# gooofy/zerovox

Hardware: AMD Instinct MI355X
Metric: audio samples/sec + RTF, 128-phoneme zero-shot synth @22.05kHz, 1/2/4/8 GPU (higher is better)
Workload: dtype f16+bf16

## Files before the change

### zerovox_amd/csrc/gemm.hip

```cpp
#include "mfma_util.h"
#include "zvx_kernels.h"

#include <cstring>
#include <type_traits>

#ifndef ZVX_GEMM_PART
#define ZVX_GEMM_PART 0
#endif
#define ZVX_PART_MAIN (ZVX_GEMM_PART != 2)
#define ZVX_PART_RESFUSE (ZVX_GEMM_PART != 1)
#if ZVX_GEMM_PART == 2
extern thread_local bool zvx_gemm_dry_run;
#else
thread_local hipEvent_t zvx_gemm_ev_start = nullptr, zvx_gemm_ev_stop = nullptr;
thread_local bool zvx_gemm_dry_run = false;
#endif
#define g_dry_run zvx_gemm_dry_run

#define ZVX_LAUNCH(...) do { if (!g_dry_run) ZVX_DISPATCH(__VA_ARGS__); } while (0)

namespace zvx {


#define PITCH 80
// ... 102 lines not shown
                }
            }
        }
    }
}

template <int DT, int BM, int BN, int WM, int WN>
__global__ __launch_bounds__(256) void gemm_kernel(const GemmArgs a) {
    constexpr int ES = (DT == DT_F32) ? 4 : 2;
    constexpr int EPC = 16 / ES;
    constexpr int BKE = KBYTES / ES;
    constexpr int TM = BM / WM / 32, TN = BN / WN / 32;
    constexpr int XCH = BM * 4 / 256;
    constexpr int WCH = (BN * 4 + 255) / 256;
    static_assert(WM * WN == 4, "4 waves");

    __shared__ __attribute__((aligned(16))) unsigned char lds[2][(BM + BN) * PITCH];

    const int tid = threadIdx.x, lane = tid & 63, wave = tid >> 6;
    const int wr = wave % WM, wc = wave / WM;

    const int ntn = (a.N + BN - 1) / BN;
    const int nwg = gridDim.x;
    int wg;
    {
        const int id = blockIdx.x, q = nwg >> 3, r = nwg & 7, xcd = id & 7;
        wg = (xcd < r ? xcd * (q + 1) : r * (q + 1) + (xcd - r) * q) + (id >> 3);
    }
    const int nt = wg % ntn, mt = wg / ntn;
    const int m0 = mt * BM, n0 = nt * BN;
    const int z = blockIdx.y, b = z / a.nheads, h = z - b * a.nheads;

    const int out_len = a.out_len ? a.out_len[b] : a.M;
    const int in_len = a.in_len ? a.in_len[b] : a.in_len_static;
    const bool two_d = a.wout > 0;
    if (!two_d && m0 >= out_len) return;
    if (m0 >= a.M) return;
    int Kb = a.K;
    if (a.k_len) { Kb = (a.k_len[b] + 7) & ~7; if (Kb > a.K) Kb = a.K; }

    const unsigned char* Xp = (const unsigned char*)a.X + ((long)b * a.x_bs + (long)h * a.x_hs) * ES;
    const unsigned char* Wp = (const unsigned char*)a.W + ((long)b * a.w_bs + (long)h * a.w_hs) * ES;

    int xu[XCH], xv[XCH];
    const int kc = tid & 3;
#pragma unroll
    for (int i = 0; i < XCH; i++) {
        const int r = m0 + (tid >> 2) + i * 64;
        if (two_d) { xu[i] = (r / a.wout) * a.stride; xv[i] = (r % a.wout) * a.stride; }
        else { xu[i] = 0; xv[i] = r; }
    }

    const int kchunks = (Kb + BKE - 1) / BKE;
    const int S = a.ntaps * kchunks;

    uint4 xreg[XCH], wreg[WCH];

    auto load_regs = [&](int s) {
        const int tap = s / kchunks;
        const int k = (s - tap * kchunks) * BKE + kc * EPC;
        const bool kok = k < Kb;
        const int du = a.du[tap], dv = a.dv[tap];
#pragma unroll
        for (int i = 0; i < XCH; i++) {
            const int iu = xu[i] + du, iv = xv[i] + dv;
            const bool ok = kok && iu >= 0 && iu < a.hin && iv >= 0 && iv < in_len;
            uint4 v = make_uint4(0, 0, 0, 0);
            if (ok) v = *(const uint4*)(Xp + ((long)(iu * a.win + iv) * a.ldx + k) * ES);
            xreg[i] = v;
        }
#pragma unroll
        for (int i = 0; i < WCH; i++) {
            const int c = tid + i * 256;
            const int n = n0 + (c >> 2);
            uint4 v = make_uint4(0, 0, 0, 0);
            if ((BN * 4 >= 256 * (i + 1) || c < BN * 4) && kok && n < a.N)
                v = *(const uint4*)(Wp + ((long)tap * a.w_ts + (long)n * a.ldw + k) * ES);
            wreg[i] = v;
        }
    };
    auto store_lds = [&](int buf) {
        unsigned char* base = lds[buf];
#pragma unroll
        for (int i = 0; i < XCH; i++)
            *(uint4*)(base + ((tid >> 2) + i * 64) * PITCH + kc * 16) = xreg[i];
#pragma unroll
        for (int i = 0; i < WCH; i++) {
            const int c = tid + i * 256;
            if (BN * 4 >= 256 * (i + 1) || c < BN * 4)
                *(uint4*)(base + (BM + (c >> 2)) * PITCH + kc * 16) = wreg[i];
        }
    };

    f32x16 acc[TN][TM];
#pragma unroll
    for (int i = 0; i < TN; i++)
#pragma unroll
        for (int j = 0; j < TM; j++)
#pragma unroll
            for (int e = 0; e < 16; e++) acc[i][j][e] = 0.f;

    const int xrow = wr * (BM / WM) + (lane & 31);
    const int wrow = BM + wc * (BN / WN) + (lane & 31);
    const int koff = (lane >> 5) * 16;

    if (S > 0) {
        load_regs(0);
        store_lds(0);
    }
    __syncthreads();
    for (int s = 0; s < S; s++) {
        if (s + 1 < S) load_regs(s + 1);
        const unsigned char* base = lds[s & 1];
#pragma unroll
        for (int sub = 0; sub < 2; sub++) {
            uint4 xf[TM], wf[TN];
#pragma unroll
            for (int j = 0; j < TM; j++) xf[j] = *(const uint4*)(base + (xrow + j * 32) * PITCH + sub * 32 + koff);
#pragma unroll
            for (int i = 0; i < TN; i++) wf[i] = *(const uint4*)(base + (wrow + i * 32) * PITCH + sub * 32 + koff);
#pragma unroll
            for (int i = 0; i < TN; i++)
#pragma unroll
                for (int j = 0; j < TM; j++) {
                    if (DT == DT_BF16) {
                        acc[i][j] = __builtin_amdgcn_mfma_f32_32x32x16_bf16(
                            __builtin_bit_cast(bf16x8, wf[i]), __builtin_bit_cast(bf16x8, xf[j]), acc[i][j], 0, 0, 0);
                    } else if (DT == DT_F16) {
                        acc[i][j] = __builtin_amdgcn_mfma_f32_32x32x16_f16(
                            __builtin_bit_cast(f16x8, wf[i]), __builtin_bit_cast(f16x8, xf[j]), acc[i][j], 0, 0, 0);
                    } else {
                        acc[i][j] = __builtin_amdgcn_mfma_f32_32x32x2f32(__uint_as_float(wf[i].x), __uint_as_float(xf[j].x), acc[i][j], 0, 0, 0);
                        acc[i][j] = __builtin_amdgcn_mfma_f32_32x32x2f32(__uint_as_float(wf[i].y), __uint_as_float(xf[j].y), acc[i][j], 0, 0, 0);
                        acc[i][j] = __builtin_amdgcn_mfma_f32_32x32x2f32(__uint_as_float(wf[i].z), __uint_as_float(xf[j].z), acc[i][j], 0, 0, 0);
                        acc[i][j] = __builtin_amdgcn_mfma_f32_32x32x2f32(__uint_as_float(wf[i].w), __uint_as_float(xf[j].w), acc[i][j], 0, 0, 0);
                    }
                }
        }
        if (s + 1 < S) store_lds((s + 1) & 1);
        __syncthreads();
    }

    epilogue<TM, TN>(a, acc, b, h, m0 + wr * (BM / WM), n0 + wc * (BN / WN), out_len, two_d, lane);
}

__device__ __forceinline__ unsigned pack_f16x2(float lo, float hi) { return pack_f16x2_sat(lo, hi); }
__device__ __forceinline__ unsigned pack16x2(float lo, float hi, bool f16) { return f16 ? pack_f16x2_sat(lo, hi) : pack_bf16x2(lo, hi); }
__device__ __forceinline__ f32x2 unpack16x2(unsigned u, bool f16) { return f16 ? unpack_f16x2(u) : unpack_bf16x2(u); }

#define ZVX_EPI(res, am, out) ((res) | ((am) << 1) | ((out) << 3))
#define ZVX_EPI_DEC(res) (16 | 8 | (res))
#define ZVX_EPI_FLIP (ZVX_EPI(0, 0, 1) | 32)

template <int TM, int TN, int RES_LDS = 0, int EPI = -1, bool H16 = false>
__device__ __forceinline__ void epilogue_rows(const GemmArgs& a, f32x16 (&acc)[TN][TM], int b, int row_base, int col_base,
                                              int out_len, int lane, unsigned char* stage ,
                                              const unsigned char* res_lds = nullptr ,
                                              int res_pitch = 0) {
    constexpr int NW = TN * 32;
    constexpr int EP = NW * 4 + 16;
    constexpr int LPR = NW / 8;
    constexpr int RPP = 64 / LPR;
    constexpr int NP = 32 / RPP;
    constexpr bool CT = EPI >= 0;
    constexpr bool DEC = CT && (EPI & 16) != 0;
    constexpr bool BURST = !(CT && !DEC && ((EPI >> 1) & 1));
    const long ooff = (long)b * a.o_bs, roff = (long)b * a.r_bs, aoff = (long)b * a.a_bs;
    const int c8 = lane % LPR;
    const int n = col_base + c8 * 8;
    const bool nok = n < a.N;
    const float alpha = CT ? 1.f : a.alpha, oscale = a.out_scale, rinv = a.res_inv_slope;
    const int act = DEC ? ACT_NONE : (CT ? ACT_LRELU : a.act);
    const float slope = CT ? (a.act == ACT_LRELU ? a.slope : 1.f) : a.slope;
    const int res_mode = RES_LDS ? 2 : (DEC ? (EPI & 1) : (CT ? ((EPI & 1) ? 2 : 0) : a.res_mode));
    const int accum_mode = DEC ? 0 : (CT ? (EPI >> 1) & 3 : a.accum_mode), bias_mode = (CT && !DEC) ? 1 : a.bias_mode;
    const bool has_out = CT ? (EPI >> 3) & 1 : a.out != nullptr, out_bf16 = CT || a.out_dtype != DT_F32, has_post = !CT && a.post_scale != nullptr;
    const bool out_f16 = CT ? H16 : a.out_dtype == DT_F16, res_f16 = (CT || RES_LDS) ? H16 : a.res_dtype == DT_F16, acc_f16 = CT ? H16 : ((TN == 1 || TM <= 2) && a.accum_dtype == DT_F16);
    const bool acc_bf16 = CT || a.accum_dtype == DT_BF16 || acc_f16, res_bf16 = CT || RES_LDS || a.res_dtype != DT_F32;
#define pk2(lo, hi, f16) ((CT && H16) ? pack_f16x2_raw(lo, hi) : pack16x2(lo, hi, f16))
    f32x2 bcol[4];
#pragma unroll
    for (int e = 0; e < 4; e++) bcol[e] = (f32x2){0.f, 0.f};
    if (bias_mode == 1 && nok) {
        const float4 b0 = *(const float4*)(a.bias + n), b1 = *(const float4*)(a.bias + n + 4);
        bcol[0] = (f32x2){b0.x, b0.y}; bcol[1] = (f32x2){b0.z, b0.w}; bcol[2] = (f32x2){b1.x, b1.y}; bcol[3] = (f32x2){b1.z, b1.w};
    }
    u32x4 pk[TM][NP];
    const bool res_glb = !RES_LDS && res_mode && res_bf16;
    uint4 rnext[NP];
    auto res_prefetch = [&](int j) {
#pragma unroll
        for (int p = 0; p < NP; p++) {
            const int r = row_base + j * 32 + p * RPP + lane / LPR;
            const bool okp = r < a.M && r < out_len && nok;
            rnext[p] = *(const uint4*)((const unsigned short*)a.res + (okp ? roff + (long)r * a.ldr + n : 0));
        }
    };
    if (res_glb) res_prefetch(0);
#pragma unroll
    for (int j = 0; j < TM; j++) {
#pragma unroll
        for (int i = 0; i < TN; i++)
#pragma unroll
            for (int g = 0; g < 4; g++)
                *(float4*)(stage + (lane & 31) * EP + (i * 32 + 8 * g + 4 * (lane >> 5)) * 4) =
                    make_float4(acc[i][j][4 * g], acc[i][j][4 * g + 1], acc[i][j][4 * g + 2], acc[i][j][4 * g + 3]);
        f32x2 v[NP][4];
        uint4 rraw[NP];
        float4 aa0[NP], aa1[NP];
        uint4 aab[NP];
        bool ok[NP];
        if (res_glb) {
#pragma unroll
            for (int p = 0; p < NP; p++) rraw[p] = rnext[p];
            if (j + 1 < TM) res_prefetch(j + 1);
        }
#pragma unroll
        for (int p = 0; p < NP; p++) {
            const int rl = p * RPP + lane / LPR;
            const int r = row_base + j * 32 + rl;
            ok[p] = r < a.M && r < out_len && nok;
            const float4 v0 = *(const float4*)(stage + rl * EP + c8 * 32), v1 = *(const float4*)(stage + rl * EP + c8 * 32 + 16);
            v[p][0] = (f32x2){v0.x, v0.y}; v[p][1] = (f32x2){v0.z, v0.w}; v[p][2] = (f32x2){v1.x, v1.y}; v[p][3] = (f32x2){v1.z, v1.w};
            if (RES_LDS == 1) rraw[p] = *(const uint4*)(res_lds + (j * 32 + rl) * res_pitch + (col_base + c8 * 8) * 2);
            if (accum_mode & 1) {
                const long ai = ok[p] ? aoff + (long)r * a.lda + n : 0;
                if (acc_bf16) aab[p] = *(const uint4*)((const unsigned short*)a.accum + ai);
                else { const float* ap = (const float*)a.accum + ai; aa0[p] = *(const float4*)ap; aa1[p] = *(const float4*)(ap + 4); }
            }
        }
#pragma unroll
        for (int p = 0; p < NP; p++) {
            const int r = row_base + j * 32 + p * RPP + lane / LPR;
            f32x2* t = v[p];
            if (alpha != 1.f) {
#pragma unroll
                for (int e = 0; e < 4; e++) t[e] *= alpha;
            }
            if (bias_mode == 1) {
#pragma unroll
                for (int e = 0; e < 4; e++) t[e] += bcol[e];
            } else if (bias_mode == 2) {
                const float brow = ok[p] ? a.bias[r] : 0.f;
#pragma unroll
                for (int e = 0; e < 4; e++) t[e] += brow;
            }
            if (res_mode) {
                f32x2 q[4];
                if (res_bf16) {
                    q[0] = unpack16x2(rraw[p].x, res_f16); q[1] = unpack16x2(rraw[p].y, res_f16); q[2] = unpack16x2(rraw[p].z, res_f16); q[3] = unpack16x2(rraw[p].w, res_f16);
                } else {
                    const float* rp = (const float*)a.res + (ok[p] ? roff + (long)r * a.ldr + n : 0);
                    const float4 t0 = *(const float4*)rp, t1 = *(const float4*)(rp + 4);
                    q[0] = (f32x2){t0.x, t0.y}; q[1] = (f32x2){t0.z, t0.w}; q[2] = (f32x2){t1.x, t1.y}; q[3] = (f32x2){t1.z, t1.w};
                }
                if (res_mode == 2) {
#pragma unroll
                    for (int e = 0; e < 4; e++) t[e] += inv_lrelu2(q[e], rinv);
                } else {
#pragma unroll
                    for (int e = 0; e < 4; e++) t[e] += q[e];
                }
            }
            if (accum_mode & 1) {
                if (acc_bf16) {
                    t[0] += unpack16x2(aab[p].x, acc_f16); t[1] += unpack16x2(aab[p].y, acc_f16); t[2] += unpack16x2(aab[p].z, acc_f16); t[3] += unpack16x2(aab[p].w, acc_f16);
                } else {
                    t[0] += (f32x2){aa0[p].x, aa0[p].y}; t[1] += (f32x2){aa0[p].z, aa0[p].w};
                    t[2] += (f32x2){aa1[p].x, aa1[p].y}; t[3] += (f32x2){aa1[p].z, aa1[p].w};
                }
            }
            if ((accum_mode & 2) && ok[p]) {
                const long ai = aoff + (long)r * a.lda + n;
                if (acc_bf16) {
                    *(u32x4*)((unsigned short*)a.accum + ai) =
                        (u32x4){pk2(t[0].x, t[0].y, acc_f16), pk2(t[1].x, t[1].y, acc_f16), pk2(t[2].x, t[2].y, acc_f16), pk2(t[3].x, t[3].y, acc_f16)};
                } else {
                    float* ap = (float*)a.accum + ai;
                    *(float4*)ap = make_float4(t[0].x, t[0].y, t[1].x, t[1].y);
                    *(float4*)(ap + 4) = make_float4(t[2].x, t[2].y, t[3].x, t[3].y);
                }
            }
            if (has_out) {
                if (DEC || (CT ? accum_mode != 0 : oscale != 1.f)) {
#pragma unroll
                    for (int e = 0; e < 4; e++) t[e] *= oscale;
                }
                if (act == ACT_LRELU) {
#pragma unroll
                    for (int e = 0; e < 4; e++) t[e] = lrelu2(t[e], slope);
                } else if (act == ACT_RELU) {
#pragma unroll
                    for (int e = 0; e < 4; e++) t[e] = (f32x2){fmaxf(t[e].x, 0.f), fmaxf(t[e].y, 0.f)};
                }
                if (has_post && nok) {
                    const float4 s0 = *(const float4*)(a.post_scale + n), s1 = *(const float4*)(a.post_scale + n + 4);
                    const float4 h0 = *(const float4*)(a.post_shift + n), h1 = *(const float4*)(a.post_shift + n + 4);
                    t[0] = t[0] * (f32x2){s0.x, s0.y} + (f32x2){h0.x, h0.y}; t[1] = t[1] * (f32x2){s0.z, s0.w} + (f32x2){h0.z, h0.w};
                    t[2] = t[2] * (f32x2){s1.x, s1.y} + (f32x2){h1.x, h1.y}; t[3] = t[3] * (f32x2){s1.z, s1.w} + (f32x2){h1.z, h1.w};
                }
                if (out_bf16) {
                    const u32x4 o = (u32x4){pk2(t[0].x, t[0].y, out_f16), pk2(t[1].x, t[1].y, out_f16), pk2(t[2].x, t[2].y, out_f16), pk2(t[3].x, t[3].y, out_f16)};
                    if (BURST) pk[j][p] = o;
                    else if (ok[p]) *(u32x4*)((unsigned short*)a.out + ooff + (long)r * a.ldo + n) = o;
                } else if (ok[p]) {
                    if (!CT && a.out_split3) {
                        unsigned short* op = (unsigned short*)a.out + ooff + (long)r * a.ldo + n;
                        u32x4 hv, lv;
#pragma unroll
                        for (int e = 0; e < 4; e++) {
                            if (a.out_split3 == 2) {
                                const unsigned hp = pack_f16x2(t[e].x, t[e].y);
                                const f32x2 rem = (t[e] - unpack_f16x2(hp)) * 2048.f;
                                hv[e] = hp; lv[e] = pack_f16x2(rem.x, rem.y);
                            } else {
                                const unsigned hp = pack_bf16x2(t[e].x, t[e].y);
                                const f32x2 rem = t[e] - unpack_bf16x2(hp);
                                hv[e] = hp; lv[e] = pack_bf16x2(rem.x, rem.y);
                            }
                        }
                        *(u32x4*)op = hv; *(u32x4*)(op + a.N) = hv; *(u32x4*)(op + 2 * a.N) = lv;
                    } else {
                        float* op = (float*)a.out + ooff + (long)r * a.ldo + n;
                        *(float4*)op = make_float4(t[0].x, t[0].y, t[1].x, t[1].y);
                        *(float4*)(op + 4) = make_float4(t[2].x, t[2].y, t[3].x, t[3].y);
                    }
                }
            }
        }
    }
    if (has_out && out_bf16 && BURST) {
        unsigned short* obase = (unsigned short*)a.out + ooff + n;
        const int ldo = a.ldo;
#pragma unroll
        for (int j = 0; j < TM; j++)
#pragma unroll
            for (int p = 0; p < NP; p++) {
                const int r = row_base + j * 32 + p * RPP + lane / LPR;
                if (r < a.M && r < out_len && nok) *(u32x4*)(obase + (long)r * ldo) = pk[j][p];
            }
    }
#undef pk2
}

template <int TM, int TN, bool F16 = false>
__device__ __forceinline__ void epilogue_direct(const GemmArgs& a, f32x16 (&acc)[TN][TM], int b, int row_base, int col_base,
                                                int out_len, int lane, unsigned char* stage ) {
    constexpr int NW = TN * 32, EP = NW * 2 + 16, LPR = NW / 8, RPP = 64 / LPR, NP = 32 / RPP;
    const float slope = a.act == ACT_LRELU ? a.slope : 1.f;
    const int h4 = 4 * (lane >> 5), c8 = lane % LPR, n = col_base + c8 * 8;
    const bool nok = n < a.N;
    float4 bb[TN][4];
#pragma unroll
    for (int i = 0; i < TN; i++)
#pragma unroll
        for (int g = 0; g < 4; g++) {
            const int co = col_base + i * 32 + 8 * g + h4;
            bb[i][g] = co < a.N ? *(const float4*)(a.bias + co) : make_float4(0.f, 0.f, 0.f, 0.f);
        }
    unsigned short* obase = (unsigned short*)a.out + (long)b * a.o_bs + n;
    u32x4 o[TM][NP];
#pragma unroll
    for (int j = 0; j < TM; j++) {
#pragma unroll
        for (int i = 0; i < TN; i++)
#pragma unroll
            for (int g = 0; g < 4; g++) {
                const f32x2 v01 = lrelu2((f32x2){acc[i][j][4 * g], acc[i][j][4 * g + 1]} + (f32x2){bb[i][g].x, bb[i][g].y}, slope);
                const f32x2 v23 = lrelu2((f32x2){acc[i][j][4 * g + 2], acc[i][j][4 * g + 3]} + (f32x2){bb[i][g].z, bb[i][g].w}, slope);
                uint2 pk;
                pk.x = pack16x2(v01.x, v01.y, F16);
                pk.y = pack16x2(v23.x, v23.y, F16);
                *(uint2*)(stage + (lane & 31) * EP + (i * 32 + 8 * g + h4) * 2) = pk;
            }
#pragma unroll
        for (int p = 0; p < NP; p++) o[j][p] = *(const u32x4*)(stage + (p * RPP + lane / LPR) * EP + c8 * 16);
    }
#pragma unroll
    for (int j = 0; j < TM; j++)
#pragma unroll
        for (int p = 0; p < NP; p++) {
            const int r = row_base + j * 32 + p * RPP + lane / LPR;
            if (r < a.M && r < out_len && nok) *(u32x4*)(obase + (long)r * a.ldo) = o[j][p];
        }
}

#if ZVX_PART_MAIN
#define SLAB_KC 64
#define SLAB_PITCH 144

__global__ void k_pack_w(const unsigned short* w, int ntaps, int N, int K, unsigned short* out, int nkc, long total_frag_lanes) {
    long idx = (long)blockIdx.x * blockDim.x + threadIdx.x;
    if (idx >= total_frag_lanes) return;
    const int lane = idx & 63; long t = idx >> 6;
    const int k16 = t & 3; t >>= 2;
    const int tap = t % ntaps; t /= ntaps;
    const int kc = t % nkc; const int nt = t / nkc;
    const int n = nt * 32 + (lane & 31);
    const int k0 = kc * SLAB_KC + k16 * 16 + 8 * (lane >> 5);
    unsigned short v[8];
#pragma unroll
    for (int e = 0; e < 8; e++) {
        const int k = k0 + e;
        v[e] = (n < N && k < K) ? w[((long)tap * N + n) * K + k] : (unsigned short)0;
    }
    uint4 o;
    o.x = v[0] | ((unsigned)v[1] << 16); o.y = v[2] | ((unsigned)v[3] << 16);
    o.z = v[4] | ((unsigned)v[5] << 16); o.w = v[6] | ((unsigned)v[7] << 16);
    *(uint4*)(out + idx * 8) = o;
}

size_t packed_weight_elems(int ntaps, int N, int K) {
    const int nkc = (K + SLAB_KC - 1) / SLAB_KC, nt = (N + 31) / 32;
    return (size_t)nt * nkc * ntaps * 4 * 64 * 8;
}
void launch_pack_weights(const void* w_bf16, int ntaps, int N, int K, void* out, hipStream_t s) {
    const int nkc = (K + SLAB_KC - 1) / SLAB_KC, nt = (N + 31) / 32;
    const long total = (long)nt * nkc * ntaps * 4 * 64;
    hipLaunchKernelGGL(k_pack_w, dim3((unsigned)((total + 255) / 256)), dim3(256), 0, s, (const unsigned short*)w_bf16, ntaps, N, K,
                       (unsigned short*)out, nkc, total);
}

void launch_pack_pair(const void* packedA, int ntapsA, int KA, const void* packedB, int ntapsB, int KB, int N, void* out, hipStream_t s) {
    const size_t nt = (N + 31) / 32;
    const size_t szA = (size_t)((KA + SLAB_KC - 1) / SLAB_KC) * ntapsA * 4 * 1024, szB = (size_t)((KB + SLAB_KC - 1) / SLAB_KC) * ntapsB * 4 * 1024;
    (void)hipMemcpy2DAsync(out, szA + szB, packedA, szA, szA, nt, hipMemcpyDeviceToDevice, s);
    (void)hipMemcpy2DAsync((char*)out + szA, szA + szB, packedB, szB, szB, nt, hipMemcpyDeviceToDevice, s);
}

template <int BM, int BN, int WM, int WN, bool FULLK, int MINW, int R, int EPI = -1, int MAXH = 64, bool F16 = false>
__global__ __launch_bounds__(256, MINW) void convslab_kernel(const GemmArgs a) {
    constexpr int TM = BM / WM / 32, TN = BN / WN / 32;
    constexpr int NIT = ((BM + MAXH) * 8 + 255) / 256;
    static_assert(WM * WN == 4, "4 waves");
    extern __shared__ __attribute__((aligned(16))) unsigned char slab[];
    if (F16 && EPI >= 0 && EPI != ZVX_EPI(0, 0, 1) && EPI != ZVX_EPI_FLIP) f16_saturate_mode();

    const int tid = threadIdx.x, lane = tid & 63, wave = __builtin_amdgcn_readfirstlane(tid >> 6);
    const int wr = wave % WM, wc = wave / WM;
    const int ntn = (a.N + BN - 1) / BN;
    int wg, b;
    if (a.xcd_flat) {
        const int nx = gridDim.x, nwg = nx * gridDim.y, id = blockIdx.y * nx + blockIdx.x, q = nwg >> 3, r = nwg & 7, xcd = id & 7;
        const int w = (xcd < r ? xcd * (q + 1) : r * (q + 1) + (xcd - r) * q) + (id >> 3);
        b = w / nx; wg = w - b * nx;
    } else {
        const int nwg = gridDim.x, id = blockIdx.x, q = nwg >> 3, r = nwg & 7, xcd = id & 7;
        wg = (xcd < r ? xcd * (q + 1) : r * (q + 1) + (xcd - r) * q) + (id >> 3);
        b = blockIdx.y;
    }
    const int nt = wg % ntn, mt = wg / ntn;
    const int m0 = mt * BM, n0 = nt * BN;
    const bool bflat = a.bflat != 0;
    const int out_len = bflat ? a.M : (a.out_len ? a.out_len[b] : a.M);
    const int in_len = bflat ? 0 : (a.in_len ? a.in_len[b] : a.in_len_static);
    if (m0 >= out_len || m0 >= a.M) return;
    if (bflat) {
        const int b0 = m0 / a.bflat, t0 = m0 - b0 * a.bflat;
        if (t0 >= a.out_len[b0] && t0 + BM <= a.bflat) return;
    }

    const int HL = a.halo_l, SR = BM + a.halo_l + a.halo_r;
    const int nkc = (a.K + SLAB_KC - 1) / SLAB_KC, n16 = a.K >> 4, ntaps = a.ntaps;
    const unsigned short* Xp = (const unsigned short*)a.X + (long)b * a.x_bs;
    const int nkc2 = (!FULLK && a.K2 > 0) ? (a.K2 + SLAB_KC - 1) / SLAB_KC : 0, n16_2 = a.K2 >> 4;
    const unsigned short* Xp2 = (const unsigned short*)a.X2 + (long)b * a.x2_bs;
    const int in_rows = ((MAXH > 64 || bflat) && a.flat_win) ? a.flat_rows : in_len;
    unsigned rowmask = 0xffffffffu;
    if (bflat) {
        rowmask = 0;
#pragma unroll
        for (int it = 0; it < NIT; it++) {
            const int g = m0 - HL + ((tid + it * 256) >> 3);
            if (g >= 0 && g < in_rows) { const int bb = g / a.bflat; if (g - bb * a.bflat < a.in_len[bb]) rowmask |= 1u << it; }
        }
    } else if (MAXH > 64 && a.flat_win) {
        rowmask = 0;
#pragma unroll
        for (int it = 0; it < NIT; it++) {
            const int g = m0 - HL + ((tid + it * 256) >> 3);
            if (g >= 0 && g < in_rows && (g % a.flat_win) < in_len) rowmask |= 1u << it;
        }
    }

    f32x16 acc[TN][TM];
#pragma unroll
    for (int i = 0; i < TN; i++)
#pragma unroll
        for (int j = 0; j < TM; j++)
#pragma unroll
            for (int e = 0; e < 16; e++) acc[i][j][e] = 0.f;

    constexpr bool WREG = R == 0;
    constexpr int F = BN / 32, CNT = F >= 4 ? F / 4 : 1, WD = 4, D = WREG ? WD : R - 1, WAITN = WREG ? (WD - 1) * TN : (D - 2) * CNT;
    const int nt32_total = (a.N + 31) >> 5;
    const int nsteps = a.ntaps * 4, gtotal = nkc * nsteps + nkc2 * 4;
    const uint4* wsrc[CNT];
#pragma unroll
    for (int j = 0; j < CNT; j++) {
        const int f = wave * CNT + j, t32 = (n0 >> 5) + f;
        wsrc[j] = (const uint4*)a.Wp + (long)(t32 < nt32_total ? t32 : 0) * gtotal * 64 + lane;
    }
    const int xrow0 = HL + wr * (BM / WM) + (lane & 31);
    const int koff = (lane >> 5) * 16;
    unsigned char* ring = slab + ((SR * SLAB_PITCH + 1023) & ~1023);
    const unsigned lds_base = (unsigned)(size_t)(__attribute__((address_space(3))) unsigned char*)slab;
    const int dvreg = a.dv[lane & (ZVX_MAX_TAPS - 1)];
    const bool loader = wave * CNT < F;
    const unsigned char* wq[TN];
#pragma unroll
    for (int i = 0; i < TN; i++) {
        const int t32 = (n0 >> 5) + wc * TN + i;
        wq[i] = (const unsigned char*)a.Wp + (long)(t32 < nt32_total ? t32 : 0) * gtotal * 1024;
    }
    const bool wave_dead = __builtin_amdgcn_readfirstlane((int)(n0 + wc * TN * 32 >= a.N)) != 0;
    const unsigned lane16 = lane * 16;
    u32x4 wreg[WREG ? WD : 1][TN] = {};
    auto wload = [&](int gs, int slot) {
        const long off = (long)(gs < gtotal ? gs : gtotal - 1) * 1024;
#pragma unroll
        for (int i = 0; i < TN; i++)
            asm volatile("global_load_dwordx4 %0, %1, %2" : "+v"(wreg[WREG ? slot : 0][i]) : "v"(lane16), "s"(wq[i] + off) : "memory");
    };
    auto dma = [&](int gs) {
        if (WREG || !loader) return;
        const int slot = gs & (R - 1);
        const long off = (long)(gs < gtotal ? gs : gtotal - 1) * 64;
#pragma unroll
        for (int j = 0; j < CNT; j++)
            __builtin_amdgcn_global_load_lds((const __attribute__((address_space(1))) void*)(wsrc[j] + off),
                                             (__attribute__((address_space(3))) void*)(ring + (slot * F + wave * CNT + j) * 1024), 16, 0, 0);
    };
    if (WREG) { wload(0, 0); wload(1, 1); wload(2, 2); wload(3, 3); }
    else {
#pragma unroll
        for (int s0 = 0; s0 < D; s0++) dma(s0);
    }

    for (int kc = 0; kc < nkc + nkc2; kc++) {
        const bool src2 = !FULLK && kc >= nkc;
        const unsigned short* const Xs = src2 ? Xp2 : Xp;
        const int ldxs = src2 ? a.ldx2 : a.ldx, Ks = src2 ? a.K2 : a.K, kbase = (src2 ? kc - nkc : kc) * SLAB_KC;
        {
            constexpr int FCH = NIT > 10 ? (NIT + 1) / 2 : NIT;
#pragma unroll
            for (int h0 = 0; h0 < NIT; h0 += FCH) {
                uint4 sv[FCH];
#pragma unroll
                for (int i = 0; i < FCH; i++) {
                    const int it = h0 + i;
                    const int c = tid + it * 256;
                    const int row = c >> 3, q = c & 7;
                    const int g = m0 - HL + row, k = kbase + q * 8;
                    sv[i] = make_uint4(0, 0, 0, 0);
                    if (it < NIT && c < SR * 8 && g >= 0 && g < in_rows && k < Ks && ((rowmask >> it) & 1)) sv[i] = *(const uint4*)(Xs + (long)g * ldxs + k);
                }
                if (kc && h0 == 0) __syncthreads();
#pragma unroll
                for (int i = 0; i < FCH; i++) {
                    const int c = tid + (h0 + i) * 256;
                    if (h0 + i < NIT && c < SR * 8) *(uint4*)(slab + (c >> 3) * SLAB_PITCH + (c & 7) * 16) = sv[i];
                }
            }
        }
        __syncthreads();
        int nk16 = 4;
        if (!FULLK) { nk16 = src2 ? n16_2 - (kc - nkc) * 4 : n16 - kc * 4; if (nk16 > 4) nk16 = 4; if (wave_dead) nk16 = 0; }
        const int ntaps_kc = src2 ? 1 : ntaps;

        uint4 xA[TM], wA[TN], xB[TM], wB[TN];
        const unsigned ring_rd = lds_base + (unsigned)(size_t)(ring - slab) + lane * 16 + wc * TN * 1024;
        const int gs0 = src2 ? nkc * nsteps + (kc - nkc) * 4 : kc * nsteps;
        auto rd = [&](uint4 (&xf)[TM], uint4 (&wf)[TN], int gs, unsigned rowoff, int kk) {
            if (!WREG) {
                const unsigned wa = ring_rd + (gs & ((WREG ? 1 : R) - 1)) * (F * 1024);
#pragma unroll
                for (int i = 0; i < TN; i++)
                    asm volatile("ds_read_b128 %0, %1 offset:%2" : "=v"(wf[i]) : "v"(wa), "n"(i * 1024));
            }
#pragma unroll
            for (int j = 0; j < TM; j++)
                asm volatile("ds_read_b128 %0, %1" : "=v"(xf[j]) : "v"(lds_base + rowoff + j * 32 * SLAB_PITCH + kk * 32));
        };
        auto mma = [&](uint4 (&xf)[TM], uint4 (&wf)[TN]) {
#pragma unroll
            for (int i = 0; i < TN; i++)
#pragma unroll
                for (int j = 0; j < TM; j++)
                    acc[i][j] = F16 ? __builtin_amdgcn_mfma_f32_32x32x16_f16(__builtin_bit_cast(f16x8, wf[i]), __builtin_bit_cast(f16x8, xf[j]), acc[i][j], 0, 0, 0)
                                    : __builtin_amdgcn_mfma_f32_32x32x16_bf16(__builtin_bit_cast(bf16x8, wf[i]),
                                                                       __builtin_bit_cast(bf16x8, xf[j]), acc[i][j], 0, 0, 0);
        };
        auto mma_r = [&](uint4 (&xf)[TM], int slot) {
#pragma unroll
            for (int i = 0; i < TN; i++)
#pragma unroll
                for (int j = 0; j < TM; j++)
                    acc[i][j] = F16 ? __builtin_amdgcn_mfma_f32_32x32x16_f16(__builtin_bit_cast(f16x8, wreg[WREG ? slot : 0][i]), __builtin_bit_cast(f16x8, xf[j]), acc[i][j], 0, 0, 0)
                                    : __builtin_amdgcn_mfma_f32_32x32x16_bf16(__builtin_bit_cast(bf16x8, wreg[WREG ? slot : 0][i]),
                                                                       __builtin_bit_cast(bf16x8, xf[j]), acc[i][j], 0, 0, 0);
        };
        auto rowoff_of = [&](int tap) {
            const int d = src2 ? 0 : __builtin_amdgcn_readlane(dvreg, tap < ntaps ? tap : ntaps - 1);
            return (unsigned)((xrow0 + d) * SLAB_PITCH + koff);
        };
        unsigned rowoff = rowoff_of(0);
        rd(xA, wA, gs0, rowoff, 0);
        for (int tap = 0; tap < ntaps_kc; tap++) {
            const unsigned rowoff_next = rowoff_of(tap + 1);
#pragma unroll
            for (int kk = 0; kk < 4; kk++) {
                const int gs = gs0 + tap * 4 + kk;
                if (WREG) asm volatile("s_waitcnt vmcnt(%0)" :: "n"(WAITN) : "memory");
                else asm volatile("s_waitcnt vmcnt(%0)\n\ts_barrier" :: "n"(WAITN) : "memory");
                dma(gs + D);
                if (kk & 1) rd(xA, wA, gs + 1, kk == 3 ? rowoff_next : rowoff, (kk + 1) & 3);
                else        rd(xB, wB, gs + 1, rowoff, kk + 1);
                asm volatile("s_waitcnt lgkmcnt(%0)" :: "n"(WREG ? TM : TM + TN) : "memory");
                __builtin_amdgcn_sched_barrier(0);
                if (FULLK || kk < nk16) {
                    if (WREG) { if (kk & 1) mma_r(xB, kk); else mma_r(xA, kk); }
                    else { if (kk & 1) mma(xB, wB); else mma(xA, wA); }
                }
                __builtin_amdgcn_sched_barrier(0);
                if (WREG) wload(gs + WD, kk);
            }
            rowoff = rowoff_next;
        }
        asm volatile("s_waitcnt lgkmcnt(0)" ::: "memory");
    }
    if (WREG) {
#pragma unroll
        for (int sl = 0; sl < (WREG ? WD : 1); sl++)
#pragma unroll
            for (int i = 0; i < TN; i++) asm volatile("s_waitcnt vmcnt(0)" : "+v"(wreg[sl][i]) :: "memory");
    } else {
        asm volatile("s_waitcnt vmcnt(0)" ::: "memory");
    }
    __syncthreads();
    if (EPI == ZVX_EPI_FLIP)
        epilogue_direct<TM, TN, !F16>(a, acc, b, m0 + wr * (BM / WM), n0 + wc * (BN / WN), out_len, lane, slab + wave * (32 * (TN * 64 + 16)));
    else if (EPI == ZVX_EPI(0, 0, 1))
        epilogue_direct<TM, TN, F16>(a, acc, b, m0 + wr * (BM / WM), n0 + wc * (BN / WN), out_len, lane, slab + wave * (32 * (TN * 64 + 16)));
    else
        epilogue_rows<TM, TN, 0, EPI, (F16 && EPI >= 0)>(a, acc, b, m0 + wr * (BM / WM), n0 + wc * (BN / WN), out_len, lane, slab + wave * (32 * (TN * 32 * 4 + 16)));
}

template <int C, int NT, int BM, int WM, int WN, int MINW, int MAXH = 64, bool F16 = false>
__global__ __launch_bounds__(256, MINW) void convreg_kernel(const GemmArgs a) {
    constexpr int TM = BM / WM / 32;
    constexpr int KS = C / 16;
    constexpr int PITCH_ = C * 2 + 16;
    constexpr int CPR = C / 8;
    constexpr int NIT = ((BM + MAXH) * CPR + 255) / 256;
    constexpr int FCH = NIT > 12 ? 8 : NIT;
    static_assert(WM * WN == 4 && WN * 32 == C, "wave layout");
    extern __shared__ __attribute__((aligned(16))) unsigned char slab[];

    const int tid = threadIdx.x, lane = tid & 63, wave = tid >> 6;
    const int wr = wave % WM, wc = wave / WM;
    int wg;
    {
        const int nwg = gridDim.x, id = blockIdx.x, q = nwg >> 3, r = nwg & 7, xcd = id & 7;
        wg = (xcd < r ? xcd * (q + 1) : r * (q + 1) + (xcd - r) * q) + (id >> 3);
    }
    const int m0 = wg * BM, b = blockIdx.y;
    const int out_len = a.out_len ? a.out_len[b] : a.M;
    const int in_len = a.in_len ? a.in_len[b] : a.in_len_static;
    if (m0 >= out_len || m0 >= a.M) return;
    const int HL = a.halo_l, SR = BM + a.halo_l + a.halo_r;
    const unsigned short* Xp = (const unsigned short*)a.X + (long)b * a.x_bs;

    uint4 w[NT][KS];
    {
        const uint4* Wq = (const uint4*)a.Wp + ((long)wc * NT * 4) * 64 + lane;
#pragma unroll
        for (int t = 0; t < NT; t++)
#pragma unroll
            for (int kk = 0; kk < KS; kk++) w[t][kk] = Wq[(t * 4 + kk) * 64];
    }
    {
        const bool flat = MAXH > 64 && a.flat_win;
        const int in_rows = flat ? a.flat_rows : in_len;
#pragma unroll
        for (int h0 = 0; h0 < NIT; h0 += FCH) {
            uint4 sv[FCH];
#pragma unroll
            for (int i = 0; i < FCH; i++) {
                const int c = tid + (h0 + i) * 256;
                const int row = c / CPR, q = c % CPR;
                const int g = m0 - HL + row;
                sv[i] = make_uint4(0, 0, 0, 0);
                if (h0 + i < NIT && c < SR * CPR && g >= 0 && g < in_rows && (!flat || (g % a.flat_win) < in_len)) sv[i] = *(const uint4*)(Xp + (long)g * a.ldx + q * 8);
            }
#pragma unroll
            for (int i = 0; i < FCH; i++) {
                const int c = tid + (h0 + i) * 256;
                if (h0 + i < NIT && c < SR * CPR) *(uint4*)(slab + (c / CPR) * PITCH_ + (c % CPR) * 16) = sv[i];
            }
        }
    }
    __syncthreads();

    f32x16 acc[1][TM];
#pragma unroll
    for (int j = 0; j < TM; j++)
#pragma unroll
        for (int e = 0; e < 16; e++) acc[0][j][e] = 0.f;
    const int xrow0 = HL + wr * (BM / WM) + (lane & 31);
    const int koff = (lane >> 5) * 16;
#pragma unroll
    for (int t = 0; t < NT; t++) {
        const unsigned char* rowp = slab + (xrow0 + a.dv[t]) * PITCH_ + koff;
#pragma unroll
        for (int kk = 0; kk < KS; kk++)
#pragma unroll
            for (int j = 0; j < TM; j++) {
                const uint4 xf = *(const uint4*)(rowp + j * 32 * PITCH_ + kk * 32);
                acc[0][j] = mfma16<F16>(w[t][kk], xf, acc[0][j]);
            }
    }
    __syncthreads();
    epilogue_rows<TM, 1>(a, acc, b, m0 + wr * (BM / WM), wc * 32, out_len, lane, slab + wave * (32 * (32 * 4 + 16)));
}

typedef __attribute__((ext_vector_type(2))) unsigned u32x2_t;
__device__ __forceinline__ void store_block_mfma_layout(unsigned short* row_ptr , const uint2 (&pk)[4], int lane, bool ok) {
#pragma unroll
    for (int pr = 0; pr < 2; pr++) {
        const u32x2_t sx = __builtin_amdgcn_permlane32_swap(pk[2 * pr].x, pk[2 * pr + 1].x, false, false);
        const u32x2_t sy = __builtin_amdgcn_permlane32_swap(pk[2 * pr].y, pk[2 * pr + 1].y, false, false);
        if (ok) *(u32x4*)(row_ptr + 8 * (2 * pr + (lane >> 5))) = (u32x4){sx.x, sy.x, sx.y, sy.y};
    }
}

template <int C, int BM, int WM, int WN, int MAXH, int MODE, int WGPC, bool POOL = false>
__global__ __launch_bounds__(WM * WN * 64, WM * WN * WGPC / 4) void conv2d_persist_kernel(const GemmArgs a, const int ntm, const int ntiles) {
    constexpr int NTHR = WM * WN * 64;
    constexpr int NT = 9, TM = BM / WM / 32, KS = C / 16, PITCH_ = C * 2 + 16, CPR = C / 8, RSTEP = NTHR / CPR;
    constexpr int NIT = ((BM + MAXH) * CPR + NTHR - 1) / NTHR;
    constexpr bool EC_LDS = NTHR > 256;
    static_assert(WN * 32 == C && BM % (WM * 32) == 0, "wave layout");
    extern __shared__ __attribute__((aligned(16))) unsigned char slab[];

    const int tid = threadIdx.x, lane = tid & 63, wave = __builtin_amdgcn_readfirstlane(tid >> 6);
    const int wr = wave % WM, wc = wave / WM;
    const int G = gridDim.x, xcd = blockIdx.x & 7, slot = blockIdx.x >> 3;
    auto tile_of = [&](int r) {
        const int base = r * G, n = ntiles - base < G ? ntiles - base : G;
        if (n <= 0) return ntiles;
        const int per = (n + 7) >> 3, t = xcd * per + slot;
        return (slot < per && t < n) ? base + t : ntiles;
    };
    const int HL = a.halo_l, SR = BM + a.halo_l + a.halo_r, win = a.flat_win, in_rows = a.flat_rows;

    uint4 w[NT][KS];
    {
        const uint4* Wq = (const uint4*)a.Wp + ((long)wc * NT * 4) * 64 + lane;
#pragma unroll
        for (int t = 0; t < NT; t++)
#pragma unroll
            for (int kk = 0; kk < KS; kk++) w[t][kk] = Wq[(t * 4 + kk) * 64];
    }
    float* const ecl = (float*)(slab + ((SR * PITCH_ + 15) & ~15));
    float4 ec0[EC_LDS ? 1 : 4], ec1[(MODE == 1 && !EC_LDS) ? 4 : 1];
    if (EC_LDS) {
        if (tid < C) { ecl[tid] = MODE == 0 ? a.bias[tid] : a.post_scale[tid]; if (MODE == 1) ecl[C + tid] = a.post_shift[tid]; }
    } else {
#pragma unroll
        for (int g = 0; g < 4; g++) {
            const int ch = wc * 32 + 8 * g + 4 * (lane >> 5);
            if (MODE == 0) ec0[g] = *(const float4*)(a.bias + ch);
            else { ec0[g] = *(const float4*)(a.post_scale + ch); ec1[g] = *(const float4*)(a.post_shift + ch); }
        }
    }
    u32x4 sv[NIT];
    const int row_t = tid / CPR, q8 = (tid % CPR) * 8;
    auto request = [&](int t) __attribute__((always_inline)) {
        const int b = t / ntm, m0 = (t - b * ntm) * BM;
        const int in_len = a.in_len[b];
        const __amdgpu_buffer_rsrc_t rs = __builtin_amdgcn_make_buffer_rsrc((void*)((const unsigned short*)a.X + (long)b * a.x_bs), 0, in_rows * a.ldx * 2, 0x00020000);
        int g = m0 - HL + row_t;
        int col = (g + 2 * win) % win;
#pragma unroll
        for (int it = 0; it < NIT; it++) {
            const bool ok = tid + it * NTHR < SR * CPR && g >= 0 && g < in_rows && col < in_len;
            sv[it] = __builtin_amdgcn_raw_buffer_load_b128(rs, ok ? (g * a.ldx + q8) * 2 : (int)0x80000000, 0, 0);
            g += RSTEP; col += RSTEP; if (col >= win) col -= win;
        }
    };
    int r = 0, t = tile_of(0);
    if (t < ntiles) request(t);
    const int xrow0 = HL + wr * (BM / WM) + (lane & 31);
    const int koff = (lane >> 5) * 16;
    constexpr bool pool = MODE == 0 && POOL;
    while (t < ntiles) {
        const int b = t / ntm, mt = t - b * ntm, m0 = mt * BM;
        if (r) asm volatile("s_waitcnt lgkmcnt(0)\n\ts_barrier" ::: "memory");
// ... 666 lines not shown
                        for (int h = 0; h < 2; h++) {
                            const int gr = qA.m0 + wrow + j * 32 + h * 16 + (lane >> 2);
                            xs[j][h] = *(const uint4*)(accp + (gr < lim ? (long)gr * a.lda : 0));
                        }
                    }
                    uint2 rrj[LEAN ? 1 : 4];
                    if (!LEAN) {
#pragma unroll
                        for (int q = 0; q < QN; q++) rrj[LEAN ? 0 : q] = *(const uint2*)(resp + j * 32 * P + q * 16);
                    }
                    uint2 pk[LEAN ? 1 : 4];
#pragma unroll
                    for (int q = 0; q < QN; q++) {
                        const float4 bq_ = LEAN ? *(const float4*)(bias2_l + wc * 32 + 8 * q + h4) : bb[LEAN ? 0 : q];
                        const uint2 rq_ = LEAN ? *(const uint2*)(resp + j * 32 * P + q * 16) : rrj[LEAN ? 0 : q];
                        f32x2 v01 = (f32x2){acc[0][j][4 * q], acc[0][j][4 * q + 1]} + (f32x2){bq_.x, bq_.y} + inv_lrelu2(unpack16<F16>(rq_.x), rinv);
                        f32x2 v23 = (f32x2){acc[0][j][4 * q + 2], acc[0][j][4 * q + 3]} + (f32x2){bq_.z, bq_.w} + inv_lrelu2(unpack16<F16>(rq_.y), rinv);
                        if (!AM) { v01 = lrelu2(v01, slope); v23 = lrelu2(v23, slope); }
                        uint2 pq;
                        pq.x = pack16<F16>(v01.x, v01.y);
                        pq.y = pack16<F16>(v23.x, v23.y);
                        if (LEAN) *(uint2*)(stage + (lane & 31) * 80 + (8 * q + h4) * 2) = pq;
                        else pk[LEAN ? 0 : q] = pq;
                    }
                    if (!LEAN) {
#pragma unroll
                        for (int q = 0; q < QN; q++) *(uint2*)(stage + (lane & 31) * 80 + (8 * q + h4) * 2) = pk[LEAN ? 0 : q];
                    }
                    uint4 o[2];
#pragma unroll
                    for (int h = 0; h < 2; h++) o[h] = *(const uint4*)(stage + (h * 16 + (lane >> 2)) * 80 + (lane & 3) * 16);
#pragma unroll
                    for (int h = 0; h < 2; h++) {
                        const int gr = qA.m0 + wrow + j * 32 + h * 16 + (lane >> 2);
                        if (AM) {
                            f32x2 t[4] = {unpack16<F16>(o[h].x), unpack16<F16>(o[h].y), unpack16<F16>(o[h].z), unpack16<F16>(o[h].w)};
                            if (AM & 1) {
                                t[0] += unpack16<F16>(xs[j][h].x); t[1] += unpack16<F16>(xs[j][h].y);
                                t[2] += unpack16<F16>(xs[j][h].z); t[3] += unpack16<F16>(xs[j][h].w);
                            }
                            if ((AM & 2) && gr < lim)
                                *(u32x4*)(accp + (long)gr * a.lda) = (u32x4){pack16<F16>(t[0].x, t[0].y), pack16<F16>(t[1].x, t[1].y),
                                                                            pack16<F16>(t[2].x, t[2].y), pack16<F16>(t[3].x, t[3].y)};
                            if (HAS_OUT) {
#pragma unroll
                                for (int e = 0; e < 4; e++) t[e] = lrelu2(t[e] * oscale, slope);
                                o[h] = make_uint4(pack16<F16>(t[0].x, t[0].y), pack16<F16>(t[1].x, t[1].y), pack16<F16>(t[2].x, t[2].y), pack16<F16>(t[3].x, t[3].y));
                            }
                        }
                        if (HAS_OUT && gr < lim) *(uint4*)(outp + (long)gr * a.ldo) = o[h];
                    }
                }
            }
        }
        asm volatile("s_waitcnt lgkmcnt(0)\n\ts_barrier" ::: "memory");
        qA = qB; qB = qC; qC = qD; qD = qE;
    }
}

template <int C, int TM = 2>
static bool launch_resfuse_persist_c(const GemmArgs& a, hipStream_t stream) {
    constexpr int BM1 = 32 * TM * (4 / (C >= 32 ? C / 32 : 1));
    const int h2 = (a.ntaps - 1) / 2, bmo = BM1 - 2 * h2;
    const int ntm = (a.M + bmo - 1) / bmo, ntiles = ntm * a.nbatch;
    const int ncu = persistent_cus();
    dim3 grid(ntiles < ncu ? ntiles : ncu);
    for (int t = 0; t < a.ntaps; t++)
        if (a.dv[t] != t - h2 || a.dv1[t] != (t - h2) * (a.dv1[1] - a.dv1[0])) return false;
    const size_t sb = ((size_t)(BM1 + 2 * a.halo_l) * (C * 2 + 16) + 1023) & ~(size_t)1023;
    const size_t tb = ((size_t)(BM1 + 2 * h2) * (C * 2 + 16) + 15) & ~(size_t)15;
    const size_t lds = 4 * sb + 2 * tb + 4 * 32 * 80 + 2 * C * 4 + 2 * 128 * 4;
    if (lds > 160 * 1024) return false;
    if (a.alpha != 1.f || a.bias_mode != 1 || a.post_scale || (a.out && a.out_dtype != a.dtype) || a.res_mode != 2 || a.res_dtype != a.dtype || a.ldo % 8 || (a.accum && (a.lda % 8 || a.accum_dtype != a.dtype))) return false;
    if (a.act != ACT_NONE && a.act != ACT_LRELU) return false;
    if (!a.accum_mode && a.out_scale != 1.f) return false;
    const int am = a.accum ? a.accum_mode : 0;
    if (!a.out && !(am & 2)) return false;
#define ZVX_RFP(NT_, AM_, HO_) if (a.dtype == DT_F16) ZVX_LAUNCH((resfuse_persist_kernel<C, NT_, AM_, HO_, TM, true>), grid, dim3(512), lds, stream, a, ntm, ntiles); else ZVX_LAUNCH((resfuse_persist_kernel<C, NT_, AM_, HO_, TM>), grid, dim3(512), lds, stream, a, ntm, ntiles); return true
#define ZVX_RFP_MODE(NT_) \
    if (a.out) { if (am == 0) { ZVX_RFP(NT_, 0, true); } if (am == 1) { ZVX_RFP(NT_, 1, true); } if (am == 2) { ZVX_RFP(NT_, 2, true); } ZVX_RFP(NT_, 3, true); } \
    else { if (am == 2) { ZVX_RFP(NT_, 2, false); } ZVX_RFP(NT_, 3, false); }
    if constexpr (TM == 1) {
        if (a.ntaps == 11) { ZVX_RFP_MODE(11) }
    } else {
        if (a.ntaps == 3) { ZVX_RFP_MODE(3) }
        if (a.ntaps == 7) { ZVX_RFP_MODE(7) }
        if constexpr (C <= 32) { if (a.ntaps == 11) { ZVX_RFP_MODE(11) } }
    }
#undef ZVX_RFP_MODE
#undef ZVX_RFP
    return false;
}

int launch_resfuse(GemmArgs a, hipStream_t stream) {
    if (a.dtype == DT_F32 || !a.Wp || !a.Wp2 || a.N != a.K || a.nheads != 1 || a.wout > 0) return -1;
    if (!(a.ntaps == 3 || a.ntaps == 7 || a.ntaps == 11)) return -1;
    int h1 = 0;
    for (int i = 0; i < a.ntaps; i++) { const int d = a.dv1[i] < 0 ? -a.dv1[i] : a.dv1[i]; if (d > h1) h1 = d; }
    if (h1 > 32) return -1;
    a.halo_l = a.halo_r = h1;
    a.fused = 1;
    if (a.N == 128 && a.no_pairstream != 1) {
        const int h2 = (a.ntaps - 1) / 2, dil = a.dv1[1] - a.dv1[0];
        bool ok = a.alpha == 1.f && a.bias_mode == 1 && !a.post_scale && (!a.out || a.out_dtype == a.dtype) && a.res_mode == 2 && a.res_dtype == a.dtype &&
                  a.res == a.X && a.r_bs == a.x_bs && a.ldr == a.ldx && (!a.accum || a.accum_dtype == a.dtype) && (a.act == ACT_NONE || a.act == ACT_LRELU) &&
                  (a.accum_mode || a.out_scale == 1.f) && a.in_len == a.out_len;
        for (int t = 0; t < a.ntaps; t++) ok = ok && a.dv[t] == t - h2 && a.dv1[t] == (t - h2) * dil;
        if (ok) {
            PairArgs p;
            memset(&p, 0, sizeof p);
            p.X = a.X; p.x_bs = a.x_bs; p.ldx = a.ldx; p.W1 = a.Wp2; p.W2 = a.Wp; p.b1 = a.bias1; p.b2 = a.bias;
            p.C = a.N; p.ntaps = a.ntaps; p.dil = dil;
            p.out = a.out; p.o_bs = a.o_bs; p.ldo = a.ldo;
            p.accum = a.accum; p.a_bs = a.a_bs; p.lda = a.lda; p.accum_mode = a.accum ? a.accum_mode : 0;
            p.slope1 = a.slope1; p.res_inv_slope = a.res_inv_slope; p.out_scale = a.out_scale; p.slope = a.act == ACT_LRELU ? a.slope : 1.f;
            p.f16 = a.dtype == DT_F16;
            p.len = a.out_len; p.M = a.M; p.nbatch = a.nbatch; p.force = a.no_pairstream == 2;
            if (launch_pairstream(p, stream, g_dry_run)) return 23;
        }
    }
    {
        if (a.N == 32 && launch_resfuse_persist_c<32>(a, stream)) return 16;
        if (a.N == 64 && a.ntaps != 11 && launch_resfuse_persist_c<64>(a, stream)) return 17;
        if (a.N == 64 && a.ntaps == 11 && launch_resfuse_persist_c<64, 1>(a, stream)) return 17;
    }
    return -1;
}
#endif
#if ZVX_PART_MAIN

struct Variant { const char* name; int dt, bm, bn; };
static const Variant kVariants[] = {
    {"gemm_bf16_128x128", DT_BF16, 128, 128}, {"gemm_bf16_256x64", DT_BF16, 256, 64},
    {"gemm_bf16_256x32", DT_BF16, 256, 32},   {"gemm_f32_128x128", DT_F32, 128, 128},
    {"gemm_f32_256x64", DT_F32, 256, 64},     {"gemm_f32_256x32", DT_F32, 256, 32},
    {"convslab_bf16_128x256", DT_BF16, 128, 256}, {"convslab_bf16_256x128", DT_BF16, 256, 128},
    {"convslab_bf16_256x64", DT_BF16, 256, 64},   {"convslab_bf16_256x32", DT_BF16, 256, 32},
    {"(unused)", DT_BF16, 0, 0}, {"resfuse_bf16_c8", DT_BF16, 256, 8}, {"resfuse_bf16_c16", DT_BF16, 256, 16}, {"resfuse_bf16_c128", DT_BF16, 64, 128},
    {"convreg_bf16_c32", DT_BF16, 512, 32},       {"convreg_bf16_c64", DT_BF16, 256, 64},
    {"resfuse_bf16_c32", DT_BF16, 256, 32},       {"resfuse_bf16_c64", DT_BF16, 128, 64},
    {"gemm_bf16_64x64", DT_BF16, 64, 64},         {"gemm_f32_64x64", DT_F32, 64, 64},
    {"resstream_bf16_c32", DT_BF16, 64, 32},      {"resstream_bf16_c64", DT_BF16, 32, 64},
    {"convslab_bf16_128x128", DT_BF16, 128, 128},
    {"pairstream_bf16_c128", DT_BF16, 128, 128},
    {"narrowstage_c16", DT_BF16, 256, 16}, {"narrowstage_c8", DT_BF16, 512, 8},
    {"conv2d_persist_c32", DT_BF16, 384, 32}, {"conv2d_persist_c64", DT_BF16, 256, 64},
    {"conv2d_s2_c32", DT_BF16, 256, 64}, {"conv2d_s2_c64", DT_BF16, 128, 128},
    {"rb2fuse_bf16_c32", DT_BF16, 256, 32}, {"rb2fuse_bf16_c64", DT_BF16, 256, 64},
};
const char* gemm_variant_name(int id) { return kVariants[id].name; }
int gemm_num_variants() { return (int)(sizeof(kVariants) / sizeof(kVariants[0])); }


template <int BM, int BN, int WM, int WN, int MINW, int R, int EPI = -1>
static void launch_slab_variant(const GemmArgs& a, dim3 grid, size_t lds, hipStream_t stream) {
    const bool fullk = a.K % SLAB_KC == 0 && a.K2 == 0;
    if constexpr (R == 0 || EPI == -1 || EPI == ZVX_EPI(0, 0, 1) || EPI == ZVX_EPI_FLIP) {
        if (a.dtype == DT_F16) {
            if (fullk) ZVX_LAUNCH((convslab_kernel<BM, BN, WM, WN, true, MINW, R, EPI, 64, true>), grid, dim3(256), lds, stream, a);
            else if constexpr (EPI != ZVX_EPI_FLIP) ZVX_LAUNCH((convslab_kernel<BM, BN, WM, WN, false, MINW, R, EPI, 64, true>), grid, dim3(256), lds, stream, a);
            return;
        }
    }
    if constexpr (EPI < 0 || !(EPI & 16)) {
        if (fullk) ZVX_LAUNCH((convslab_kernel<BM, BN, WM, WN, true, MINW, R, EPI>), grid, dim3(256), lds, stream, a);
        else if constexpr (EPI != ZVX_EPI_FLIP) ZVX_LAUNCH((convslab_kernel<BM, BN, WM, WN, false, MINW, R, EPI>), grid, dim3(256), lds, stream, a);
    }
}

int gemm_epi_mode_of(const GemmArgs& a) {
    if (a.alpha == 1.f && !a.post_scale && a.out && a.out_dtype != a.dtype && a.dtype != DT_F32 && a.out_dtype != DT_F32 && !a.out_split3 && a.bias_mode == 1 && a.bias &&
        (a.act == ACT_NONE || a.act == ACT_LRELU) && !a.res_mode && !(a.accum && a.accum_mode) && a.out_scale == 1.f && a.K % SLAB_KC == 0 && !a.K2) return ZVX_EPI_FLIP;
    if (a.alpha != 1.f || a.post_scale || (a.out && a.out_dtype != a.dtype) || a.dtype == DT_F32 || a.out_split3 || a.bias_mode == 2) return -1;
    const int am = a.accum ? a.accum_mode : 0;
    if (a.dtype == DT_F16 && a.out && !am && a.act == ACT_NONE && a.res_mode <= 1 && (!a.res_mode || a.res_dtype == DT_F16) && (a.res_mode || a.out_scale != 1.f) &&
        (a.bias_mode == 0 || a.bias)) return ZVX_EPI_DEC(a.res_mode ? 1 : 0);
    if (a.bias_mode != 1 || !a.bias) return -1;
    if (a.act != ACT_NONE && a.act != ACT_LRELU) return -1;
    if (a.res_mode && (a.res_mode != 2 || a.res_dtype != a.dtype)) return -1;
    if (am && a.accum_dtype != a.dtype) return -1;
    if (!am && a.out_scale != 1.f) return -1;
    if (!a.out && !(am & 2)) return -1;
    const int e = ZVX_EPI(a.res_mode ? 1 : 0, am, a.out ? 1 : 0);
    switch (e) {
        case ZVX_EPI(0, 0, 1): case ZVX_EPI(1, 0, 1): case ZVX_EPI(1, 2, 0): case ZVX_EPI(1, 3, 0): case ZVX_EPI(1, 1, 1): return e;
    }
    return -1;
}

static int launch_convslab(GemmArgs a, hipStream_t stream) {
    const bool bflat_hint = a.bflat != 0;
    if (a.K2) {
        if (!a.X2 || a.K2 % 16 || a.ldx2 % 8 || a.flat_win || (a.bflat && a.x2_bs != (long)a.bflat * a.ldx2)) return -5;
    }
    if (a.bflat) {
        int h = 0;
        for (int i = 0; i < a.ntaps; i++) { const int d = a.dv[i] < 0 ? -a.dv[i] : a.dv[i]; if (d > h) h = d; }
        const bool ok = a.in_len && a.out_len && a.nbatch > 1 && a.bflat >= a.M + h && a.x_bs == (long)a.bflat * a.ldx && (!a.out || a.o_bs == (long)a.bflat * a.ldo) &&
                        (!a.res_mode || a.r_bs == (long)a.bflat * a.ldr) && !a.accum_mode && a.bias_mode != 2 && !a.flat_win && a.M > 128 && a.N >= 128 &&
                        (long)a.nbatch * a.bflat < (1l << 30);
        if (!ok) a.bflat = 0;
    }
    const int g_slab_small = a.slab_small & 7;
    int hl = 0, hr = 0;
    for (int i = 0; i < a.ntaps; i++) { hl = a.dv[i] < -hl ? -a.dv[i] : hl; hr = a.dv[i] > hr ? a.dv[i] : hr; }
    a.halo_l = hl; a.halo_r = hr;
    if (a.flat_win && !a.bflat) {
        if (a.N == a.K && (a.N == 32 || a.N == 64) && !(a.slab_small & 32) && a.dtype == DT_BF16 && a.ntaps == 9 && a.in_len && !a.out_len && hl == a.flat_win + 1 && hr == hl &&
            a.flat_win >= 64 && (long)a.flat_rows * a.ldx * 2 < 0x7fffffffL &&
            a.out && a.out_dtype == DT_BF16 && a.alpha == 1.f && a.out_scale == 1.f && !a.res_mode && !a.accum_mode && !a.out_split3 && a.ldo % 8 == 0 &&
            ((a.post_scale && a.post_shift && a.bias_mode == 0 && a.act == ACT_RELU) || (!a.post_scale && a.bias_mode == 1 && a.bias && a.act == ACT_NONE))) {
            if (a.N == 32 && hl + hr <= 544) { launch_conv2d_persist<32, 384, 4, 1, 544, 2>(a, stream); return 26; }
            if (a.N == 64 && hl + hr <= 288) { launch_conv2d_persist<64, 256, 4, 2, 288, 1>(a, stream); return 27; }
        }
        if (a.N == a.K && a.N == 32 && launch_convreg_c<32, 384, 4, 1, 2>(a, stream)) return 14;
        if (a.N == a.K && a.N == 64 && launch_convreg_c<64, 256, 2, 2, 2>(a, stream)) return 15;
        if (a.N % 128 || a.K % SLAB_KC || hl + hr > 160) return -4;
        const int pad256 = ((a.M + 255) / 256) * 256, pad128 = ((a.M + 127) / 128) * 128;
        if ((long)pad256 * 100 > (long)pad128 * 115) {
            dim3 g128((a.N / 128) * (pad128 / 128), a.nbatch);
            size_t lds128 = ((size_t)(128 + hl + hr) * SLAB_PITCH + 1023) & ~(size_t)1023;
            const size_t stage128 = (size_t)4 * 32 * (2 * 128 + 16);
            if (lds128 < stage128) lds128 = stage128;
            ZVX_LAUNCH((convslab_kernel<128, 128, 2, 2, true, 2, 0, -1, 160>), g128, dim3(256), lds128, stream, a);
            return 22;
        }
        dim3 grid((a.N / 128) * ((a.M + 255) / 256), a.nbatch);
        size_t lds = ((size_t)(256 + hl + hr) * SLAB_PITCH + 1023) & ~(size_t)1023;
        ZVX_LAUNCH((convslab_kernel<256, 128, 2, 2, true, 2, 0, -1, 160>), grid, dim3(256), lds, stream, a);
        return 7;
    }
    if (a.dtype != DT_F32 && a.N == a.K && !a.K2 && (a.ntaps == 3 || a.ntaps == 5 || a.ntaps == 7 || a.ntaps == 11)) {
        if (a.N == 32 && launch_convreg_c<32, 512, 4, 1, 2>(a, stream)) return 14;
        if (a.N == 64 && launch_convreg_c<64, 256, 2, 2, 2>(a, stream)) return 15;
    }
    if (hl + hr > 64) {
        if (hl + hr <= 160 && a.N % 128 == 0 && a.K % SLAB_KC == 0 && !a.K2 && !a.bflat && !a.flat_win && gemm_epi_mode_of(a) == ZVX_EPI(1, 1, 1)) {
            dim3 grid((a.N / 128) * ((a.M + 255) / 256), a.nbatch);
            const size_t lds = ((size_t)(256 + hl + hr) * SLAB_PITCH + 1023) & ~(size_t)1023;
            if (a.dtype == DT_F16) ZVX_LAUNCH((convslab_kernel<256, 128, 2, 2, true, 2, 0, ZVX_EPI(1, 1, 1), 160, true>), grid, dim3(256), lds, stream, a);
            else ZVX_LAUNCH((convslab_kernel<256, 128, 2, 2, true, 2, 0, ZVX_EPI(1, 1, 1), 160>), grid, dim3(256), lds, stream, a);
            return 7;
        }
        return -4;
    }
    static const int bns[4] = {256, 128, 64, 32};
    static const double eff[4] = {0.95, 1.0, 0.7, 0.4};
    int best = 0; double best_cost = -1;
    for (int i = 0; i < 4; i++) {
        const double cost = (double)((a.N + bns[i] - 1) / bns[i]) * bns[i] / eff[i];
        if (best_cost < 0 || cost < best_cost - 1e-9) { best_cost = cost; best = i; }
    }
    static const int bms[4] = {128, 256, 256, 256};
    const int ncu = num_cus();
    if (g_slab_small >= 2 && a.M <= 64 && a.nbatch * ((a.N + 127) / 128) * 4 <= ncu && a.N >= 64 && hl + hr <= 64) {
        a.bflat = 0;
        dim3 g32((a.N + 31) / 32, a.nbatch);
        const size_t lds32 = (((size_t)(256 + hl + hr) * SLAB_PITCH + 1023) & ~(size_t)1023) + (size_t)8 * 1024;
        launch_slab_variant<256, 32, 4, 1, 2, 8>(a, g32, lds32, stream);
        return 9;
    }
    if (g_slab_small && a.M > 128 && a.N >= 128 && hl + hr <= 64) {
        const long wg256 = (long)((a.N + 127) / 128) * ((a.M + 255) / 256) * a.nbatch;
        if (wg256 * 2 <= ncu) {
            a.bflat = 0;
            const bool r64 = wg256 * 4 <= ncu;
            const int bm = r64 ? 64 : 128;
            dim3 gs(((a.N + 127) / 128) * ((a.M + bm - 1) / bm), a.nbatch);
            size_t lds = ((size_t)(bm + hl + hr) * SLAB_PITCH + 1023) & ~(size_t)1023;
            const size_t stage = (size_t)4 * 32 * (2 * 128 + 16);
            if (lds < stage) lds = stage;
            if (r64) launch_slab_variant<64, 128, 2, 2, 2, 0>(a, gs, lds, stream);
            else launch_slab_variant<128, 128, 2, 2, 2, 0>(a, gs, lds, stream);
            return 22;
        }
    }
    if (a.M <= 128 && a.N >= 128) {
        a.bflat = 0;
        const int wide = ((a.N + 255) / 256) * a.nbatch;
        const bool narrow = wide < 2 * ncu;
        const int bn = narrow ? 128 : 256;
        dim3 grid((a.N + bn - 1) / bn, a.nbatch);
        size_t lds = ((size_t)(128 + hl + hr) * SLAB_PITCH + 1023) & ~(size_t)1023;
        const size_t stage = (size_t)4 * 32 * (2 * 128 + 16);
        if (lds < stage) lds = stage;
        if (narrow && a.M > (g_slab_small ? 32 : 64) && ((a.N + 127) / 128) * a.nbatch < 2 * ncu) {
            dim3 g64(((a.N + 127) / 128) * ((a.M + 63) / 64), a.nbatch);
            launch_slab_variant<64, 128, 2, 2, 2, 0>(a, g64, lds, stream);
            return 22;
        }
        if (narrow) { launch_slab_variant<128, 128, 2, 2, 2, 0>(a, grid, lds, stream); return 22; }
        launch_slab_variant<128, 256, 1, 4, 2, 0>(a, grid, lds, stream);
        return 6;
    }
    if (a.ntaps == 1 && a.N >= 512) {
        const long slots = 2L * ncu;
        auto rounds = [&](int bm_, int bn_) {
            const long ntn_ = (a.N + bn_ - 1) / bn_, utt = ntn_ * ((a.M + bm_ - 1) / bm_) * a.nbatch;
            const long flat = a.bflat ? ntn_ * (((long)a.nbatch * a.bflat + bm_ - 1) / bm_) : utt;
            return ((flat < utt ? flat : utt) + slots - 1) / slots;
        };
        best = rounds(256, 128) <= rounds(128, 256) ? 1 : 0;
    }
    const bool wreg = best <= 1;
    const int ring_slots = wreg ? 0 : (best == 0 ? 4 : 8);
    const int bn = bns[best], bm = bms[best];
    const int ntn = (a.N + bn - 1) / bn;
    if (a.bflat) {
        const long slots = 2L * ncu;
        const long wg_utt = (long)ntn * ((a.M + bm - 1) / bm) * a.nbatch, wg_flat = (long)ntn * (((long)a.nbatch * a.bflat + bm - 1) / bm);
        if ((wg_flat + slots - 1) / slots < (wg_utt + slots - 1) / slots) { a.flat_win = a.bflat; a.flat_rows = a.nbatch * a.bflat; a.M = a.flat_rows; a.nbatch = 1; }
        else a.bflat = 0;
    }
    if (best == 1 && bflat_hint && a.M > 256 && hl + hr <= 64) {
        const long slots = 2L * ncu;
        const long t256 = (long)ntn * ((a.M + 255) / 256) * a.nbatch, t128 = (long)ntn * ((a.M + 127) / 128) * a.nbatch;
        const long eff256 = 2 * ((t256 + slots - 1) / slots), eff128 = (t128 + slots - 1) / slots;
        if (eff128 < eff256) {
            dim3 g128(ntn * ((a.M + 127) / 128), a.nbatch);
            size_t lds128 = ((size_t)(128 + hl + hr) * SLAB_PITCH + 1023) & ~(size_t)1023;
            const size_t stage128 = (size_t)4 * 32 * (2 * 128 + 16);
            if (lds128 < stage128) lds128 = stage128;
            switch (gemm_epi_mode_of(a)) {
                case ZVX_EPI(0, 0, 1): launch_slab_variant<128, 128, 2, 2, 2, 0, ZVX_EPI(0, 0, 1)>(a, g128, lds128, stream); break;
                case ZVX_EPI_DEC(0): launch_slab_variant<128, 128, 2, 2, 2, 0, ZVX_EPI_DEC(0)>(a, g128, lds128, stream); break;
                case ZVX_EPI_DEC(1): launch_slab_variant<128, 128, 2, 2, 2, 0, ZVX_EPI_DEC(1)>(a, g128, lds128, stream); break;
                default: launch_slab_variant<128, 128, 2, 2, 2, 0>(a, g128, lds128, stream);
            }
            return 22;
        }
    }
    const int ntm = (a.M + bm - 1) / bm;
    dim3 grid(ntn * ntm, a.nbatch);
    const int tn = (bn >= 128) ? 2 : 1;
    if (a.accum_mode && a.accum && a.accum_dtype == DT_F16 && tn == 2 && !(best == 1 && gemm_epi_mode_of(a) >= 0)) return -6;
    size_t lds = (((size_t)(bm + hl + hr) * SLAB_PITCH + 1023) & ~(size_t)1023) + (size_t)ring_slots * (bn / 32) * 1024;
    const size_t stage = (size_t)4 * 32 * (tn * 128 + 16);
    if (lds < stage) lds = stage;
    switch (best) {
        case 0: launch_slab_variant<128, 256, 1, 4, 2, 0>(a, grid, lds, stream); break;
        case 1: switch (gemm_epi_mode_of(a)) {
                    case ZVX_EPI(0, 0, 1): launch_slab_variant<256, 128, 2, 2, 2, 0, ZVX_EPI(0, 0, 1)>(a, grid, lds, stream); break;
                    case ZVX_EPI_FLIP: launch_slab_variant<256, 128, 2, 2, 2, 0, ZVX_EPI_FLIP>(a, grid, lds, stream); break;
                    case ZVX_EPI(1, 0, 1): launch_slab_variant<256, 128, 2, 2, 2, 0, ZVX_EPI(1, 0, 1)>(a, grid, lds, stream); break;
                    case ZVX_EPI(1, 2, 0): launch_slab_variant<256, 128, 2, 2, 2, 0, ZVX_EPI(1, 2, 0)>(a, grid, lds, stream); break;
                    case ZVX_EPI(1, 3, 0): launch_slab_variant<256, 128, 2, 2, 2, 0, ZVX_EPI(1, 3, 0)>(a, grid, lds, stream); break;
                    case ZVX_EPI(1, 1, 1): launch_slab_variant<256, 128, 2, 2, 2, 0, ZVX_EPI(1, 1, 1)>(a, grid, lds, stream); break;
                    case ZVX_EPI_DEC(0): launch_slab_variant<256, 128, 2, 2, 2, 0, ZVX_EPI_DEC(0)>(a, grid, lds, stream); break;
                    case ZVX_EPI_DEC(1): launch_slab_variant<256, 128, 2, 2, 2, 0, ZVX_EPI_DEC(1)>(a, grid, lds, stream); break;
                    default: launch_slab_variant<256, 128, 2, 2, 2, 0>(a, grid, lds, stream);
                }
                break;
        case 2: launch_slab_variant<256, 64, 2, 2, 2, 8>(a, grid, lds, stream); break;
        case 3: launch_slab_variant<256, 32, 4, 1, 2, 8>(a, grid, lds, stream); break;
    }
    return 6 + best;
}


int launch_gemm(const GemmArgs& a, hipStream_t stream) {
    if (a.N <= 0 || a.M <= 0 || a.nbatch <= 0) return -1;
    if (a.ds_out) return launch_conv2d_s2(a, stream) ? 28 : -7;
    if (a.stride == 2 && a.wout > 0 && a.ntaps == 9 && a.K == 64 && a.Wp && launch_conv2d_s2(a, stream)) return 29;
    if (a.ntaps < 1 || a.ntaps > ZVX_MAX_TAPS) return -2;
    if (a.out_split3 && (a.out_dtype != DT_F32 || a.N % 8 || a.flat_win || a.wout > 0)) return -2;
    if (a.N % 4 && (a.bias_mode == 1 || a.res_mode || a.accum_mode || a.post_scale || a.ldo < ((a.N + 3) & ~3))) return -2;
    if (a.Wp && a.dtype == DT_BF16 && a.wout > 0 && a.stride == 1 && a.ntaps == 9 && a.wout == a.win && a.M == a.hin * a.win && a.nheads == 1 && a.w_bs == 0 &&
        !a.k_len && a.K % 16 == 0 && a.N % 32 == 0 && a.ldo % 8 == 0 && a.ldx == a.K && !a.res_mode && !a.accum_mode && a.bias_mode != 2 && a.win <= 271) {
        bool ok9 = true;
        for (int t = 0; t < 9; t++) ok9 = ok9 && a.du[t] == t / 3 - 1 && a.dv[t] == t % 3 - 1;
        if (ok9 && (a.N == a.K ? (a.N == 32 || a.N == 64 || (a.N % 128 == 0 && 2 * (a.win + 1) <= 160)) : false)) {
            GemmArgs f = a;
            f.flat_win = a.win; f.flat_rows = a.hin * a.win;
            for (int t = 0; t < 9; t++) { f.dv[t] = a.du[t] * a.win + a.dv[t]; f.du[t] = 0; }
            f.wout = 0; f.out_len = nullptr;
            const int id = launch_convslab(f, stream);
            if (id >= 0) return id;
        }
    }
    if (a.Wp && a.dtype != DT_F32 && a.wout <= 0 && a.nheads == 1 && a.w_bs == 0 && !a.k_len && a.K % 16 == 0 && a.N % 8 == 0 && a.ldo % 8 == 0) {
        int lo = 0, hi = 0;
        for (int i = 0; i < a.ntaps; i++) { if (a.dv[i] < lo) lo = a.dv[i]; if (a.dv[i] > hi) hi = a.dv[i]; }
        if (hi - lo <= 64 && hi >= 0 && lo <= 0) return launch_convslab(a, stream);
        if (hi - lo <= 96 && hi >= 0 && lo <= 0 && a.ntaps == 7 && a.N == a.K && (a.N == 32 || a.N == 64 || a.N == 128) && !a.K2 && !a.out_split3 && !a.bflat) {
            const int id = launch_convslab(a, stream);
            if (id >= 0) return id;
        }
    }
    if (a.out_split3 || a.K2) return -2;
    static const int bns[3] = {128, 64, 32};
    static const double eff[3] = {1.0, 0.75, 0.45};
    int best = 0; double best_cost = -1;
    for (int i = 0; i < 3; i++) {
        const double cost = (double)((a.N + bns[i] - 1) / bns[i]) * bns[i] / eff[i];
        if (best_cost < 0 || cost < best_cost - 1e-9) { best_cost = cost; best = i; }
    }
    int bn = bns[best], bm = (bn == 128) ? 128 : 256;
    int ntn = (a.N + bn - 1) / bn, ntm = (a.M + bm - 1) / bm;
    if ((long)ntn * ntm * a.nbatch * a.nheads < 512 && a.N >= 64) {
        bm = bn = 64; ntn = (a.N + 63) / 64; ntm = (a.M + 63) / 64;
        dim3 grid(ntn * ntm, a.nbatch * a.nheads), block(256);
        if (a.dtype == DT_BF16) { ZVX_LAUNCH((gemm_kernel<DT_BF16, 64, 64, 2, 2>), grid, block, 0, stream, a); return 18; }
        if (a.dtype == DT_F16) { ZVX_LAUNCH((gemm_kernel<DT_F16, 64, 64, 2, 2>), grid, block, 0, stream, a); return 18; }
        ZVX_LAUNCH((gemm_kernel<DT_F32, 64, 64, 2, 2>), grid, block, 0, stream, a);
        return 19;
    }
    dim3 grid(ntn * ntm, a.nbatch * a.nheads), block(256);
    const int base = (a.dtype != DT_F32) ? 0 : 3;
    const int id = base + best;
    if (a.dtype == DT_F16) {
        switch (id) {
            case 0: ZVX_LAUNCH((gemm_kernel<DT_F16, 128, 128, 2, 2>), grid, block, 0, stream, a); break;
            case 1: ZVX_LAUNCH((gemm_kernel<DT_F16, 256, 64, 4, 1>), grid, block, 0, stream, a); break;
            case 2: ZVX_LAUNCH((gemm_kernel<DT_F16, 256, 32, 4, 1>), grid, block, 0, stream, a); break;
        }
        return id;
    }
    switch (id) {
        case 0: ZVX_LAUNCH((gemm_kernel<DT_BF16, 128, 128, 2, 2>), grid, block, 0, stream, a); break;
        case 1: ZVX_LAUNCH((gemm_kernel<DT_BF16, 256, 64, 4, 1>), grid, block, 0, stream, a); break;
        case 2: ZVX_LAUNCH((gemm_kernel<DT_BF16, 256, 32, 4, 1>), grid, block, 0, stream, a); break;
        case 3: ZVX_LAUNCH((gemm_kernel<DT_F32, 128, 128, 2, 2>), grid, block, 0, stream, a); break;
        case 4: ZVX_LAUNCH((gemm_kernel<DT_F32, 256, 64, 4, 1>), grid, block, 0, stream, a); break;
        case 5: ZVX_LAUNCH((gemm_kernel<DT_F32, 256, 32, 4, 1>), grid, block, 0, stream, a); break;
    }
    return id;
}

int gemm_variant_of(const GemmArgs& a) {
    g_dry_run = true;
    const int id = a.fused == 2 ? launch_rb2fuse(a, nullptr) : (a.fused ? launch_resfuse(a, nullptr) : launch_gemm(a, nullptr));
    g_dry_run = false;
    return id;
}

#endif
}
```

### zerovox_amd/csrc/zvx.hip

```cpp
#include "../../include/zvx.h"
#include "zvx_kernels.h"

#include <dlfcn.h>
#include <math.h>
#include <cmath>
#include <rccl/rccl.h>
#include <stdarg.h>
#include <stdio.h>
#include <string.h>

#include <algorithm>
#include <map>
#include <sstream>
#include <stdexcept>
#include <string>
#include <vector>

using namespace zvx;

namespace {

struct ZvxError : std::runtime_error {
    int code;
    ZvxError(int c, const std::string& m) : std::runtime_error(m), code(c) {}
};
[[noreturn]] void fail(int code, const char* fmt, ...) {
    char buf[512];
    va_list ap; va_start(ap, fmt); vsnprintf(buf, sizeof buf, fmt, ap); va_end(ap);
    throw ZvxError(code, buf);
}
#define HIPCHK(x) do { hipError_t e_ = (x); if (e_ != hipSuccess) fail(ZVX_E_HIP, "%s failed: %s (%s:%d)", #x, hipGetErrorString(e_), __FILE__, __LINE__); } while (0)

thread_local std::string g_create_error;

struct Tensor {
    char kind = 'p';
    std::vector<int> dims;
    size_t off = 0, numel = 0;
    void* dev = nullptr;
    int dtype = DT_F32;
    const float* host = nullptr;
    float alpha = 1.f;
    int dim(int i) const { return dims.at(i); }
};

struct DevBuf { void* p = nullptr; void* base = nullptr; size_t cap = 0; };

struct GemmEvent { hipEvent_t a, b; int variant; double flops, bytes; long rows; int N, K, taps, res, fused; std::string tag, kname; };

}

struct zvx_ctx {
    int device = 0;
    hipStream_t stream = nullptr;
    hipStream_t main0 = nullptr;
    hipStream_t comm_stream = nullptr;
    hipStream_t voc_aux[2] = {nullptr, nullptr};
    hipEvent_t voc_ev[3] = {nullptr, nullptr, nullptr};
    int voc_overlap_maxb = 1 << 20;
    int voc_overlap_frames = 28672;
    hipStream_t front_stream = nullptr;
    hipEvent_t ev_front_done = nullptr, ev_mel_free = nullptr, ev_main_join = nullptr;
    int front_overlap = 1;
    bool mel_free_pending = false;
    bool front_dirty_main = true;
    struct HostSlot { void* p = nullptr; size_t cap = 0; hipEvent_t ready = nullptr, done = nullptr; bool pending = false; int B = 0, pcm16 = 0; long stride = 0, need = 0; };
    HostSlot host_slot[2];
    int host_next = 0, host_last = -1;
    hipStream_t copy_stream = nullptr;
    bool copy_is_comm = false;
    hipStream_t aux_stream = nullptr;
    hipEvent_t ev_aux[2] = {nullptr, nullptr};
    int va_overlap_maxb = 1 << 20;
    ncclComm_t comm = nullptr;
    int rank = 0, world = 1;
    hipEvent_t ev_compute = nullptr;
    std::map<const void*, hipEvent_t> gather_fence;
    std::string err;
    std::map<std::string, std::string> cfg;
    std::map<std::string, Tensor> tensors;
    std::vector<float> host_blob;
    std::map<std::string, DevBuf> bufs;
    std::map<const void*, const void*> packed;
    std::map<const void*, const void*> pair_packed;
    int dt = DT_BF16;
    int H = 0, emb_dim = 0, punct_dim = 0, n_phone_rows = 0, n_punct_rows = 0, max_txt_len = 0, max_mel_len = 0;
    int enc_layers = 0, enc_heads = 0, ffn_dim = 0, ffn_k0 = 0, ffn_k1 = 0, vp_dim = 0, vp_k = 0, n_bins = 0;
    int dec_layers = 0, dec_heads = 0, dec_scln = 0, n_mels = 0, hop = 0, res_dim = 0, dec_kind = 0, rn_asp = 1;
    std::vector<int> rn_layers, rn_filters, voc_rates, voc_ksizes, voc_rb_k;
    std::vector<std::vector<int>> voc_rb_d;
    int voc_resblock = 1, voc_c0 = 0;
    int B = 0, Tmax = 0, Lmax = 0;
    std::vector<int> T_host, mel_len_host;
    std::vector<int> in_stage;
    bool have_features = false, have_mel = false;
    int profile = 0;
    int profile_only = -1;
    int rs_prof = 0;
    int enc_split = 0;
    const void* fft_xs_ready = nullptr;
    int norm_fuse_maxb = 1 << 20;
    int dec_sc_fuse = 1;
    int dec_flat = 1;
    int voc_f16_stages = -1;
    int voc_h16_ok = -1;
    int voc_f16 = 1;
    int dec_f16 = 1;
    int use_attn_f32 = 1;
    int use_flash = 1;
    int use_resstream = 1;
    int rs_seg_min = 0;
    int spk_s2_fuse = 1;
    int spk_pool_fuse = 1;
    int slab_small = 2, slab_flat = 1;
    int poison_pads = 0;
    int sat_check = 0;
    unsigned long long* sat_count_dev() { return (unsigned long long*)buf("sat.count", 64); }
    void sat_scan(const void* x, int dt, long bs, int ld, int B, int rows_max, const int* rows, int C) {
        if (sat_check && x && dt == DT_F16) launch_count_sat16(x, bs, ld, B, rows_max, rows, C, sat_count_dev(), stream);
    }
    int use_rb2fuse = 1;
    int use_stagefuse = 1;
    struct NsWeights { void* W = nullptr; float* bias = nullptr; int woff[18] = {0}; };
    std::map<std::string, NsWeights> ns_weights;
    int use_pairstream = 1;
    int shape_log = 0;
    int max_frames = 1 << 18;
    int out_rate = 0;
    struct RsBank { int L = 0, M = 0, half = 0, T = 0, pitch = 0; const float* dev = nullptr; };
    std::map<std::pair<int, int>, RsBank> rs_banks;
    std::map<int, const double*> lim_wins;
    std::map<int, LoudCoef> loud_coefs;
    struct DnTables { int n_fft = 0, log2n = 0, win_length = 0; const float* twid = nullptr; const float* win = nullptr; const double* win2 = nullptr; double den_min = 0; };
    DnTables dn_tab;
    void* join_host = nullptr;
    size_t join_host_cap = 0;
    void* join_pinned(size_t bytes) {
        if (bytes > join_host_cap) {
            if (join_host) { HIPCHK(hipStreamSynchronize(stream)); HIPCHK(hipHostFree(join_host)); join_host = nullptr; join_host_cap = 0; }
            const size_t cap = bytes + bytes / 8 + 256;
            HIPCHK(hipHostMalloc(&join_host, cap, hipHostMallocDefault));
            join_host_cap = cap;
        }
        return join_host;
    }
    hipEvent_t stage_ev[ZVX_T_COUNT][2];
    bool stage_used[ZVX_T_COUNT];
    float stage_ms[ZVX_T_COUNT];
    std::vector<GemmEvent> pending;
    std::vector<zvx_kernel_stat> stats;
    std::string tag = "other";
    std::map<std::string, zvx_kernel_stat> tagstats;
    std::map<std::string, zvx_kernel_stat> namedstats;
    std::vector<hipEvent_t> event_pool;

    int cfg_int(const char* k) const {
        auto it = cfg.find(k);
        if (it == cfg.end()) fail(ZVX_E_MANIFEST, "manifest: missing cfg '%s'", k);
        return atoi(it->second.c_str());
    }
    std::vector<int> cfg_list(const char* k) const {
        auto it = cfg.find(k);
        if (it == cfg.end()) fail(ZVX_E_MANIFEST, "manifest: missing cfg '%s'", k);
        std::vector<int> v; std::stringstream ss(it->second); std::string tok;
        while (std::getline(ss, tok, ',')) if (!tok.empty()) v.push_back(atoi(tok.c_str()));
        return v;
    }
    const Tensor& t(const std::string& name) const {
        auto it = tensors.find(name);
        if (it == tensors.end()) fail(ZVX_E_MANIFEST, "weights: tensor '%s' missing", name.c_str());
        return it->second;
    }
    bool has(const std::string& name) const { return tensors.count(name) != 0; }
    const float* pf(const std::string& name) const { return (const float*)t(name).dev; }

    void drain_for_free() {
        HIPCHK(hipStreamSynchronize(stream));
        for (hipStream_t s2 : {main0, front_stream, aux_stream, voc_aux[0], voc_aux[1], comm_stream, copy_stream})
            if (s2 && s2 != stream) HIPCHK(hipStreamSynchronize(s2));
    }
    void* buf(const std::string& name, size_t bytes) {
        DevBuf& d = bufs[name];
        if (bytes > d.cap) {
            if (d.base) { drain_for_free(); HIPCHK(hipFree(d.base)); d.base = nullptr; d.p = nullptr; }
            size_t cap = bytes + bytes / 8 + 256;
            HIPCHK(hipMalloc(&d.base, cap));
            HIPCHK(hipMemsetAsync(d.base, 0, cap, stream));
            d.p = d.base;
            d.cap = cap;
        }
        return d.p;
    }
    char* carve(const std::string& pool, const std::vector<std::string>& names, size_t bytes_each, size_t* stride_out) {
        const size_t stride = (bytes_each + 255) & ~(size_t)255;
        char* base = (char*)buf(pool, stride * names.size());
        for (size_t i = 0; i < names.size(); i++) {
            DevBuf& d = bufs[names[i]];
            if (d.base) { drain_for_free(); HIPCHK(hipFree(d.base)); d.base = nullptr; }
            d.p = base + i * stride; d.cap = stride;
        }
        *stride_out = stride;
        return base;
    }
    int* ibuf(const std::string& name, size_t n) { return (int*)buf(name, n * sizeof(int)); }
    float* fbuf(const std::string& name, size_t n) { return (float*)buf(name, n * sizeof(float)); }
    struct Arena { char* p = nullptr; size_t cap = 0, cur = 0; hipEvent_t ev = nullptr; bool pending = false; };
    Arena arena[2];
    int arena_i = 0;
    int api_depth = 0;
    static constexpr size_t ARENA_BYTES = 2u << 20;
    void arena_begin() {
        Arena& a = arena[arena_i];
        if (a.pending) { HIPCHK(hipEventSynchronize(a.ev)); a.pending = false; }
        a.cur = 0;
    }
    void arena_end() {
        Arena& a = arena[arena_i];
        if (!a.cur || !stream) return;
        if (!a.ev) HIPCHK(hipEventCreateWithFlags(&a.ev, hipEventDisableTiming));
        HIPCHK(hipEventRecord(a.ev, stream));
        a.pending = true;
        arena_i ^= 1;
    }
    void upload(void* dst, const void* src, size_t bytes) {
        Arena& a = arena[arena_i];
        const size_t need = (bytes + 63) & ~(size_t)63;
        if (!a.p) { HIPCHK(hipHostMalloc((void**)&a.p, ARENA_BYTES, hipHostMallocDefault)); a.cap = ARENA_BYTES; }
        if (a.cur + need > a.cap) {
            HIPCHK(hipMemcpyAsync(dst, src, bytes, hipMemcpyHostToDevice, stream));
            HIPCHK(hipStreamSynchronize(stream));
            return;
        }
        memcpy(a.p + a.cur, src, bytes);
        HIPCHK(hipMemcpyAsync(dst, a.p + a.cur, bytes, hipMemcpyHostToDevice, stream));
        a.cur += need;
    }
    int* upload_ints(const std::string& name, const int* v, size_t n) {
        int* d = ibuf(name, n);
        upload(d, v, n * sizeof(int));
        return d;
    }
    size_t es() const { return dtype_size(dt); }

    hipEvent_t new_event() {
        hipEvent_t e;
        if (!event_pool.empty()) { e = event_pool.back(); event_pool.pop_back(); return e; }
        HIPCHK(hipEventCreate(&e));
        return e;
    }
    void stage_begin(int s) { if (profile) { HIPCHK(hipEventRecord(stage_ev[s][0], stream)); } }
    void stage_end(int s) { if (profile) { HIPCHK(hipEventRecord(stage_ev[s][1], stream)); stage_used[s] = true; } }

    template <typename V, typename L, typename D>
    void profiled(V&& vid, L&& launch, D&& describe) {
        const bool prof = profile >= 2 && (profile_only < 0 || vid() == profile_only);
        if (!prof) { launch(); return; }
        GemmEvent ev{};
        ev.a = new_event(); ev.b = new_event();
        struct Armed { Armed(hipEvent_t a, hipEvent_t b) { profile_events(a, b); } ~Armed() { profile_events(nullptr, nullptr); } };
        ev.variant = [&] { Armed armed(ev.a, ev.b); return launch(); }();
        describe(ev);
        ev.tag = tag;
        pending.push_back(ev);
    }
    void gemm(GemmArgs& a) {
        if (a.flops <= 0) a.flops = 2.0 * (double)a.M * a.nbatch * a.nheads * (double)a.N * ((double)a.K * a.ntaps + (double)a.K2);
        if (!a.Wp && a.dtype != DT_F32) { auto it = packed.find(a.W); if (it != packed.end()) a.Wp = it->second; }
        a.slab_small = slab_small | (spk_s2_fuse ? 0 : 32); a.xcd_flat = slab_flat;
        profiled([&] { return gemm_variant_of(a); }, [&] {
            const int id = a.fused == 2 ? launch_rb2fuse(a, stream) : (a.fused ? launch_resfuse(a, stream) : launch_gemm(a, stream));
            if (id < 0) fail(ZVX_E_INVALID, "launch_gemm rejected shape M=%d N=%d K=%d taps=%d", a.M, a.N, a.K, a.ntaps);
            return id;
        }, [&](GemmEvent& ev) {
            ev.flops = a.flops; ev.rows = (long)a.M * a.nbatch * a.nheads; ev.N = a.N; ev.K = a.K; ev.taps = a.ntaps; ev.res = a.res_mode; ev.fused = a.fused;
            const double esz = dtype_size(a.dtype);
            const double cells = (double)a.M * a.nbatch * a.nheads * a.N;
            ev.bytes = ((double)a.M * a.nbatch * a.nheads) * (double)(a.K + a.K2) * esz + (double)a.N * ((double)a.K * a.ntaps + a.K2) * esz * (a.fused ? 2 : 1) +
                       (a.out ? cells * dtype_size(a.out_dtype) : 0.0) + ((a.res_mode && !a.fused) ? cells * dtype_size(a.res_dtype) : 0.0) +
                       ((a.accum && (a.accum_mode & 1)) ? cells * dtype_size(a.accum_dtype) : 0.0) + ((a.accum && (a.accum_mode & 2)) ? cells * dtype_size(a.accum_dtype) : 0.0);
        });
        if (sat_check && a.nheads == 1) {
            sat_scan(a.out, a.out_dtype, a.o_bs, a.ldo, a.nbatch, a.M, a.out_len, a.N);
            if (a.accum && (a.accum_mode & 2)) sat_scan(a.accum, a.accum_dtype, a.a_bs, a.lda, a.nbatch, a.M, a.out_len, a.N);
        }
    }
    bool run_stream(StreamArgs& a) {
        const int id = launch_resstream(a, this->stream, true);
        if (id < 0) return false;
        profiled([&] { return id; }, [&] {
            const int id2 = launch_resstream(a, this->stream, false);
            if (id2 < 0) fail(ZVX_E_INVALID, "launch_resstream rejected a shape its dry run accepted (C=%d k=%d pairs=%d)", a.C, a.ntaps, a.npair);
            return id2;
        }, [&](GemmEvent& ev) {
            const double rows = (double)a.M * a.nbatch;
            ev.flops = 2.0 * 2.0 * a.npair * rows * a.C * a.C * a.ntaps; ev.rows = (long)rows; ev.N = a.C; ev.K = a.C; ev.taps = a.ntaps;
            ev.res = a.accum_mode; ev.fused = 10 + a.npair;
            ev.bytes = rows * a.C * 2.0 * (1 + (a.out ? 1 : 0) + ((a.accum && (a.accum_mode & 1)) ? 1 : 0) + ((a.accum && (a.accum_mode & 2)) ? 1 : 0));
        });
        return true;
    }
    template <typename F>
    void timed(double flops, double bytes, F&& f, const char* kname = nullptr) {
        const bool prof = profile >= 2 && profile_only < 0;
        GemmEvent ev{};
        if (prof) { ev.a = new_event(); ev.b = new_event(); HIPCHK(hipEventRecord(ev.a, stream)); }
        f();
        if (prof) { HIPCHK(hipEventRecord(ev.b, stream)); ev.variant = -1; ev.flops = flops; ev.bytes = bytes; ev.tag = tag; if (kname) ev.kname = kname; pending.push_back(ev); }
    }
    void resolve_events() {
        if (stats.empty()) {
            stats.resize(gemm_num_variants());
            for (int i = 0; i < gemm_num_variants(); i++) { memset(&stats[i], 0, sizeof stats[i]); snprintf(stats[i].name, 64, "%s", gemm_variant_name(i)); }
        }
        for (auto& e : pending) {
            float ms = 0.f;
            HIPCHK(hipEventElapsedTime(&ms, e.a, e.b));
            if (shape_log && e.variant >= 0) fprintf(stderr, "launch %-24s rows=%-8ld N=%-4d K=%-4d taps=%-2d res=%d fused=%d  %8.3f ms %8.1f TF/s %8.1f GB/s(alg)\n",
                                   gemm_variant_name(e.variant), e.rows, e.N, e.K, e.taps, e.res, e.fused, ms, e.flops / ms / 1e9, e.bytes / ms / 1e6);
            else if (shape_log) fprintf(stderr, "launch %-24s [%s]  %8.3f ms %8.1f GB/s(alg)\n", "(helper)", e.tag.c_str(), ms, e.bytes / ms / 1e6);
            if (e.variant >= 0) { auto& s = stats[e.variant]; s.launches++; s.ms += ms; s.flops += e.flops; s.bytes += e.bytes; }
            auto& ts = tagstats[e.tag];
            if (!ts.name[0]) snprintf(ts.name, 64, "%s", e.tag.c_str());
            ts.launches++; ts.ms += ms; ts.flops += e.flops; ts.bytes += e.bytes;
            if (!e.kname.empty()) {
                auto& ks = namedstats[e.kname];
                if (!ks.name[0]) snprintf(ks.name, 64, "%s", e.kname.c_str());
                ks.launches++; ks.ms += ms; ks.flops += e.flops; ks.bytes += e.bytes;
            }
            event_pool.push_back(e.a); event_pool.push_back(e.b);
        }
        pending.clear();
        for (int s = 0; s < ZVX_T_COUNT; s++)
            if (stage_used[s]) { float ms = 0.f; HIPCHK(hipEventElapsedTime(&ms, stage_ev[s][0], stage_ev[s][1])); stage_ms[s] = ms; stage_used[s] = false; }
    }
    void sync() {
        if (front_stream) HIPCHK(hipStreamSynchronize(front_stream));
        HIPCHK(hipStreamSynchronize(stream));
        if (comm_stream) HIPCHK(hipStreamSynchronize(comm_stream));
        if (copy_stream && !copy_is_comm) HIPCHK(hipStreamSynchronize(copy_stream));
        if (profile) resolve_events();
    }
    void quiesce_side_streams() noexcept {
        if (front_stream) (void)hipStreamSynchronize(front_stream);
        if (aux_stream) (void)hipStreamSynchronize(aux_stream);
        for (int i = 0; i < 2; i++) if (voc_aux[i]) (void)hipStreamSynchronize(voc_aux[i]);
        front_dirty_main = true; mel_free_pending = false;
    }
    void front_setup() {
        if (front_stream) return;
        int least = 0, greatest = 0;
        HIPCHK(hipDeviceGetStreamPriorityRange(&least, &greatest));
        HIPCHK(hipStreamCreateWithPriority(&front_stream, hipStreamNonBlocking, greatest));
        HIPCHK(hipEventCreateWithFlags(&ev_front_done, hipEventDisableTiming));
        HIPCHK(hipEventCreateWithFlags(&ev_mel_free, hipEventDisableTiming));
        HIPCHK(hipEventCreateWithFlags(&ev_main_join, hipEventDisableTiming));
    }
};

namespace {

GemmArgs gemm_base(int dtype) {
    GemmArgs a;
    memset(&a, 0, sizeof a);
    a.dtype = dtype; a.nbatch = 1; a.nheads = 1; a.ntaps = 1; a.stride = 1; a.wout = 0; a.hin = 1; a.win = 0;
    a.alpha = 1.f; a.out_scale = 1.f; a.out_dtype = dtype; a.res_dtype = dtype;
    return a;
}
void set_taps_1d(GemmArgs& a, int k, int dilation) {
    a.ntaps = k;
    for (int i = 0; i < k; i++) { a.du[i] = 0; a.dv[i] = (int)((i - (k - 1) / 2) * dilation); }
}

void parse_manifest(zvx_ctx* c, const char* manifest, const void* weights, size_t nbytes) {
    if (!manifest || !weights) fail(ZVX_E_MANIFEST, "manifest/weights pointer is NULL");
    const size_t nfloats = nbytes / 4;
    c->host_blob.assign((const float*)weights, (const float*)weights + nfloats);
    std::stringstream ss(manifest);
    std::string line;
    bool first = true;
    while (std::getline(ss, line)) {
        if (line.empty()) continue;
        std::stringstream ls(line);
        std::string kw; ls >> kw;
        if (first) { if (kw != "zvx_manifest") fail(ZVX_E_MANIFEST, "manifest: bad magic '%s'", kw.c_str()); first = false; continue; }
        if (kw == "cfg") {
            std::string k, v; ls >> k; std::getline(ls, v);
            size_t p = v.find_first_not_of(' ');
            c->cfg[k] = p == std::string::npos ? "" : v.substr(p);
        } else if (kw == "tensor") {
            std::string name, kind; int nd = 0; ls >> name >> kind >> nd;
            Tensor t; t.kind = kind.empty() ? 'p' : kind[0]; t.numel = 1;
            for (int i = 0; i < nd; i++) { int d; ls >> d; t.dims.push_back(d); t.numel *= (size_t)d; }
            ls >> t.off;
            if (ls.fail() || t.off + t.numel > nfloats) fail(ZVX_E_MANIFEST, "manifest: tensor '%s' out of blob bounds", name.c_str());
            c->tensors[name] = t;
        } else {
            fail(ZVX_E_MANIFEST, "manifest: unknown line '%s'", line.c_str());
        }
    }
    if (first) fail(ZVX_E_MANIFEST, "manifest: empty");
}

void build_split_weights(zvx_ctx* c, bool f16) {
    const char* sfx = f16 ? ".s3h" : ".s3";
    if (c->has(std::string("enc.0.wqk") + sfx)) return;
    std::vector<std::pair<std::string, Tensor>> add;
    size_t stotal = 0;
    for (auto& kv : c->tensors) {
        const Tensor& t = kv.second;
        const bool mine = kv.first.rfind("enc.", 0) == 0;
        if (!mine || t.kind != 'f' || t.dtype != DT_F32 || t.dims.size() != 3 || (3 * t.dim(2)) % 16 || t.dim(1) % 8) continue;
        Tensor s3 = t;
        s3.kind = 's'; s3.dtype = f16 ? DT_F16 : DT_BF16; s3.dims = {t.dim(0), t.dim(1), 3 * t.dim(2)}; s3.numel = t.numel * 3; s3.host = nullptr;
        stotal += ((s3.numel * 2 + 255) & ~(size_t)255) + ((packed_weight_elems(s3.dim(0), s3.dim(1), s3.dim(2)) * 2 + 255) & ~(size_t)255);
        add.emplace_back(kv.first + sfx, s3);
    }
    char* sarena = stotal ? (char*)c->buf(f16 ? "weights_split_h" : "weights_split", stotal) : nullptr;
    float* mx_d = f16 ? c->fbuf("weights_split_absmax", 64) : nullptr;
    size_t soff = 0;
    for (auto& kv : add) {
        Tensor& s3 = kv.second;
// ... 824 lines not shown
    a.X = v.A; a.x_bs = (long)rows_in * Cin; a.ldx = Cin; a.ldw = Cin;
    a.M = rows_in; a.K = Cin; a.nbatch = B; a.in_len = s.len_in; a.out_len = s.len_in;
    a.bias_mode = 1; a.act = ACT_LRELU; a.slope = 0.1f;
    a.o_bs = (long)rows_in * u * Cout; a.ldo = u * Cout;
    if (dt_in != DT_F32 && c->has(up + "_wlo")) {
        const int hc = (u / 2) * Cout;
        a.N = hc; a.ntaps = 2; a.w_ts = (long)hc * Cin; a.flops = 2.0 * B * (double)rows_in * Cin * Cout * ku / 2;
        a.W = voc_weight(c, up + "_wlo", dt_in).dev; a.dv[0] = -1; a.dv[1] = 0;
        a.bias = c->pf(up + "_b"); a.out = v.X0;
        c->gemm(a);
        a.Wp = nullptr;
        a.W = voc_weight(c, up + "_whi", dt_in).dev; a.dv[0] = 0; a.dv[1] = 1;
        a.bias = c->pf(up + "_b") + hc; a.out = (char*)v.X0 + (size_t)hc * c->es();
        c->gemm(a);
    } else {
        a.W = voc_weight(c, up + "_w", dt_in).dev; a.w_ts = (long)u * Cout * Cin; a.N = u * Cout;
        a.ntaps = 3; a.dv[0] = -1; a.dv[1] = 0; a.dv[2] = 1;
        a.bias = c->pf(up + "_b"); a.out = v.X0;
        a.flops = 2.0 * B * (double)rows_in * Cin * Cout * ku;
        c->gemm(a);
    }
}

const zvx_ctx::NsWeights& voc_narrow_weights(zvx_ctx* c, const VocCall& v, const VocStage& s) {
    const int Cout = s.Cout, nk = v.nk;
    const std::string key = "voc.ns." + std::to_string(s.i) + (s.dt == DT_F16 ? ".h16" : "");
    auto it = c->ns_weights.find(key);
    if (it != c->ns_weights.end()) return it->second;
    zvx_ctx::NsWeights nw;
    int nfrag = 0;
    for (int j = 0; j < nk; j++) for (int q = 0; q < 6; q++) { nw.woff[6 * j + q] = nfrag; nfrag += narrowstage_steps(Cout, c->voc_rb_k[j]); }
    nw.W = c->buf(key + ".w", (size_t)nfrag * 1024);
    nw.bias = c->fbuf(key + ".b", (size_t)6 * nk * Cout);
    for (int j = 0; j < nk; j++) {
        const RbWeights w = voc_rb_weights(c, v, s, j);
        for (int t = 0; t < 3; t++)
            for (int q = 0; q < 2; q++) {
                const RbConv& cv = q ? w.c2[t] : w.c1[t];
                if (cv.w->dims.size() != 3 || cv.w->dim(0) != c->voc_rb_k[j] || cv.w->dim(1) != Cout || cv.w->dim(2) != Cout) fail(ZVX_E_MANIFEST, "weights: '%s' has an unexpected shape", cv.name.c_str());
                const int ci = 6 * j + 2 * t + q;
                launch_pack_narrow(cv.w->dev, c->voc_rb_k[j], Cout, (char*)nw.W + (size_t)nw.woff[ci] * 1024, c->stream);
                HIPCHK(hipMemcpyAsync(nw.bias + (size_t)ci * Cout, cv.bias, (size_t)Cout * 4, hipMemcpyDeviceToDevice, c->stream));
            }
    }
    return c->ns_weights.emplace(key, nw).first->second;
}

bool voc_narrow_stage(zvx_ctx* c, const VocCall& v, const VocStage& s) {
    const int Cout = s.Cout, nk = v.nk, rows = s.rows;
    if (!c->use_stagefuse || c->sat_check || c->voc_resblock != 1 || s.dt == DT_F32 || (Cout != 16 && Cout != 8) || nk < 1 || nk > 3) return false;
    for (int j = 0; j < nk; j++) if (c->voc_rb_d[j].size() != 3) return false;
    const zvx_ctx::NsWeights& nw = voc_narrow_weights(c, v, s);
    StageArgs sa;
    memset(&sa, 0, sizeof sa);
    sa.X = v.X0; sa.x_bs = (long)rows * Cout; sa.ldx = Cout; sa.W = nw.W; sa.bias = nw.bias;
    memcpy(sa.woff, nw.woff, sizeof sa.woff);
    sa.C = Cout; sa.nk = nk;
    for (int j = 0; j < nk; j++) { sa.ks[j] = c->voc_rb_k[j]; for (int t = 0; t < 3; t++) sa.dil[j][t] = c->voc_rb_d[j][t]; }
    sa.out = v.A; sa.o_bs = (long)rows * Cout; sa.ldo = Cout;
    sa.slope1 = 0.1f; sa.res_inv_slope = 10.0f; sa.slope = s.next_slope;
    sa.len = s.len; sa.M = rows; sa.nbatch = v.B; sa.f16 = s.dt == DT_F16;
    if (!launch_narrowstage(sa, c->stream, true)) return false;
    const int vid = Cout == 16 ? 24 : 25;
    c->profiled([&] { return vid; }, [&] {
        if (!launch_narrowstage(sa, c->stream, false)) fail(ZVX_E_INVALID, "launch_narrowstage rejected a stage its dry run accepted (C=%d)", Cout);
        return vid;
    }, [&](GemmEvent& ev) {
        double ksum = 0; for (int j = 0; j < nk; j++) ksum += c->voc_rb_k[j];
        const double rws = (double)rows * v.B;
        ev.flops = 2.0 * rws * Cout * Cout * 6.0 * ksum; ev.rows = (long)rws; ev.N = Cout; ev.K = Cout; ev.taps = (int)ksum; ev.fused = 100 + nk;
        ev.bytes = rws * Cout * 2.0 * 2.0;
    });
    return true;
}

void voc_side_begin(zvx_ctx* c) {
    for (int q = 0; q < 2; q++) if (!c->voc_aux[q]) HIPCHK(hipStreamCreateWithFlags(&c->voc_aux[q], hipStreamNonBlocking));
    for (int q = 0; q < 3; q++) if (!c->voc_ev[q]) HIPCHK(hipEventCreateWithFlags(&c->voc_ev[q], hipEventDisableTiming));
    HIPCHK(hipEventRecord(c->voc_ev[0], c->stream));
}
struct SideHop {
    zvx_ctx* const c; hipStream_t const main_stream, aux; hipEvent_t const done; bool on_aux = false;
    SideHop(zvx_ctx* c_, hipStream_t aux_, hipEvent_t done_) : c(c_), main_stream(c_->stream), aux(aux_), done(done_) {
        if (aux) HIPCHK(hipStreamWaitEvent(aux, c->voc_ev[0], 0));
    }
    ~SideHop() { c->stream = main_stream; }
    void to_aux() { if (aux && !on_aux) { c->stream = aux; on_aux = true; } }
    void to_main() {
        if (on_aux) {
            HIPCHK(hipEventRecord(done, aux));
            c->stream = main_stream; on_aux = false;
            HIPCHK(hipStreamWaitEvent(main_stream, done, 0));
        }
    }
};

void voc_resblock(zvx_ctx* c, const VocCall& v, const VocStage& s, int j) {
    const int B = v.B, rows = s.rows, Cout = s.Cout, dt = s.dt;
    const bool side = v.side_ok && j >= 1;
    SideHop hop(c, side ? c->voc_aux[j - 1] : nullptr, side ? c->voc_ev[j] : nullptr);
    void* const T1s = side ? v.sideT1[j - 1] : v.T1;
    void* const* const PPs = side ? v.sidePP[j - 1] : v.PP;
    const int k = c->voc_rb_k[j];
    const std::vector<int>& dil = c->voc_rb_d[j];
    const int nd = (int)dil.size();
    const RbWeights w = voc_rb_weights(c, v, s, j);
    const StageClose close = stage_close(j, v.nk);
    const void* cur = v.X0;
    int pp = 0;
    int t_first = 0;
    if (c->voc_resblock == 1 && dt != DT_F32 && c->use_resstream && !c->sat_check && nd >= 1 && nd <= 3) {
        bool packed_ok = true;
        for (int t = 0; t < nd; t++) packed_ok = packed_ok && w.c1[t].packed && w.c2[t].packed;
        auto chain = [&](int t0, int np, const void* in, bool closes) {
            StreamArgs sa;
            memset(&sa, 0, sizeof sa);
            sa.X = in; sa.x_bs = (long)rows * Cout; sa.ldx = Cout; sa.C = Cout; sa.ntaps = k; sa.npair = np;
            for (int q = 0; q < np; q++) {
                sa.W1[q] = w.c1[t0 + q].packed; sa.W2[q] = w.c2[t0 + q].packed;
                sa.b1[q] = w.c1[t0 + q].bias; sa.b2[q] = w.c2[t0 + q].bias;
                sa.dil[q] = dil[t0 + q];
            }
            sa.seg_min = c->rs_seg_min; sa.f16 = dt == DT_F16;
            if (c->rs_prof) sa.prof = (long long*)c->buf("rs.prof." + w.name + "." + std::to_string(t0), 16 * 16 * 8);
            sa.slope1 = 0.1f; sa.res_inv_slope = 10.0f; sa.out_scale = 1.f; sa.slope = 0.1f;
            sa.len = s.len; sa.M = rows; sa.nbatch = B; sa.o_bs = (long)rows * Cout; sa.ldo = Cout; sa.a_bs = (long)rows * Cout; sa.lda = Cout;
            if (closes) close_stage(sa, close, v, s);
            else sa.out = PPs[pp];
            return sa;
        };
        if (packed_ok) {
            StreamArgs whole = chain(0, nd, v.X0, true);
            hop.to_main();
            if (c->run_stream(whole)) t_first = nd;
            else if (nd == 3) {
                StreamArgs head = chain(0, 2, v.X0, false);
                StreamArgs probe = chain(2, 1, PPs[pp], true);
                if (launch_resstream(head, c->stream, true) >= 0 && launch_resstream(probe, c->stream, true) >= 0) {
                    hop.to_aux();
                    c->run_stream(head);
                    cur = PPs[pp]; pp ^= 1;
                    StreamArgs tail = chain(2, 1, cur, true);
                    hop.to_main();
                    c->run_stream(tail);
                    t_first = nd;
                }
            }
        }
    }
    auto rb_base = [&] {
        GemmArgs a = gemm_base(dt);
        a.M = rows; a.N = Cout; a.K = Cout; a.nbatch = B; a.in_len = s.len; a.out_len = s.len; a.ldw = Cout; a.w_ts = (long)Cout * Cout;
        a.x_bs = (long)rows * Cout; a.ldx = Cout; a.o_bs = (long)rows * Cout; a.ldo = Cout;
        return a;
    };
    if (c->voc_resblock == 2 && nd == 2 && dt != DT_F32 && c->use_rb2fuse && !c->sat_check && (Cout == 32 || Cout == 64) && w.c1[0].packed && w.c1[1].packed) {
        GemmArgs a = rb_base();
        a.X = v.X0; a.W = w.c1[1].w->dev; a.Wp = w.c1[1].packed; a.Wp2 = w.c1[0].packed;
        a.bias1 = w.c1[0].bias; a.slope1 = 0.1f; a.fused = 2;
        set_taps_1d(a, k, dil[1]);
        for (int q = 0; q < k; q++) a.dv1[q] = (q - (k - 1) / 2) * dil[0];
        a.bias = w.c1[1].bias; a.bias_mode = 1;
        a.res = v.X0; a.r_bs = (long)rows * Cout; a.ldr = Cout; a.res_mode = 2; a.res_inv_slope = 10.0f; a.res_dtype = dt;
        close_stage(a, close, v, s);
        a.flops = 2.0 * 2.0 * B * (double)rows * Cout * Cout * k;
        if (gemm_variant_of(a) >= 0) { hop.to_main(); c->gemm(a); t_first = nd; }
    }
    for (int t = t_first; t < nd; t++) {
        const bool last = (t == nd - 1);
        if (last) hop.to_main(); else hop.to_aux();
        auto rb_tail = [&](GemmArgs& a) {
            a.bias_mode = 1;
            a.res = cur; a.r_bs = (long)rows * Cout; a.ldr = Cout; a.res_mode = 2; a.res_inv_slope = 10.0f; a.res_dtype = dt;
            if (last) close_stage(a, close, v, s);
            else { a.act = ACT_LRELU; a.slope = 0.1f; a.out = PPs[pp]; }
        };
        GemmArgs a = rb_base();
        if (c->voc_resblock == 1) {
            const RbConv& c1 = w.c1[t]; const RbConv& c2 = w.c2[t];
            bool fuse = dt != DT_F32 && !c->sat_check && c1.packed && c2.packed;
            if (fuse) {
                a.X = cur; a.W = c2.w->dev; a.Wp = c2.packed; a.Wp2 = c1.packed;
                a.bias1 = c1.bias; a.slope1 = 0.1f; a.fused = 1;
                a.no_pairstream = c->use_pairstream <= 0 ? 1 : (c->use_pairstream == 3 ? 2 : 0);
                set_taps_1d(a, k, 1);
                for (int q = 0; q < k; q++) a.dv1[q] = (q - (k - 1) / 2) * dil[t];
                a.bias = c2.bias;
                a.flops = 2.0 * 2.0 * B * (double)rows * Cout * Cout * k;
                rb_tail(a);
                const int fv = gemm_variant_of(a);
                fuse = fv >= 0 && !(Cout == 128 && fv != 23);
            }
            if (!fuse) {
                a = rb_base();
                a.X = cur; a.W = c1.w->dev;
                set_taps_1d(a, k, dil[t]);
                a.bias = c1.bias; a.bias_mode = 1; a.act = ACT_LRELU; a.slope = 0.1f;
                a.out = T1s;
                c->gemm(a);
                a = rb_base();
                a.X = T1s; a.W = c2.w->dev;
                set_taps_1d(a, k, 1);
                a.bias = c2.bias;
                rb_tail(a);
            }
        } else {
            a.X = cur; a.W = w.c1[t].w->dev;
            set_taps_1d(a, k, dil[t]);
            a.bias = w.c1[t].bias;
            rb_tail(a);
        }
        c->gemm(a);
        if (!last) { cur = PPs[pp]; pp ^= 1; }
    }
}

void run_vocoder(zvx_ctx* c, const float* mel, int ldm, int Lmel_max, const int* mel_len_host, const int* P_host, int B,
                 void* wav_dev, long wav_stride, int pcm16) {
    const std::vector<int> dom = voc_domains(c);
    const int nm = c->n_mels;
    const size_t es = dtype_size(c->dt);
    int Pmax = 0; for (int b = 0; b < B; b++) Pmax = std::max(Pmax, P_host[b]);
    if (Pmax <= 0) return;
    const int ns = (int)c->voc_rates.size(), nk = (int)c->voc_rb_k.size();
    std::vector<int> lens((size_t)(ns + 2) * B);
    for (int b = 0; b < B; b++) { lens[b] = mel_len_host[b]; lens[B + b] = P_host[b]; }
    int mul = 1;
    for (int i = 0; i < ns; i++) { mul *= c->voc_rates[i]; for (int b = 0; b < B; b++) lens[(size_t)(i + 2) * B + b] = P_host[b] * mul; }
    VocCall v{};
    v.B = B; v.Pmax = Pmax; v.nk = nk;
    v.lens_d = c->upload_ints("voc.lens", lens.data(), lens.size());
    const int* mel_len_d = v.lens_d; const int* P_d = v.lens_d + B;

    size_t maxel = (size_t)Pmax * c->voc_c0; mul = 1;
    for (int i = 0; i < ns; i++) { mul *= c->voc_rates[i]; maxel = std::max(maxel, (size_t)Pmax * mul * (size_t)(c->voc_c0 >> (i + 1))); }
    maxel *= B;
    void* vin = c->buf("voc.in", (size_t)B * Pmax * nm * es);
    v.A = c->buf("voc.A", maxel * es);
    v.X0 = c->buf("voc.X0", maxel * es);
    v.T1 = c->buf("voc.T1", maxel * es);
    v.PP[0] = c->buf("voc.PP0", maxel * es); v.PP[1] = c->buf("voc.PP1", maxel * es);
    v.XS = c->buf("voc.XS", maxel * es);
    v.side_ok = nk >= 2 && nk <= 3 && B <= c->voc_overlap_maxb && (long)B * Pmax < c->voc_overlap_frames;
    if (v.side_ok)
        for (int j = 1; j < nk; j++) {
            v.sideT1[j - 1] = c->buf("voc.T1." + std::to_string(j), maxel * es);
            v.sidePP[j - 1][0] = c->buf("voc.PP0." + std::to_string(j), maxel * es); v.sidePP[j - 1][1] = c->buf("voc.PP1." + std::to_string(j), maxel * es);
        }

    c->tag = "voc.pre";
    launch_mel_pad(mel, DT_F32, ldm, Lmel_max, mel_len_d, vin, dom[0], nm, Pmax, P_d, B, nm, c->stream);
    c->sat_scan(vin, dom[0], (long)Pmax * nm, nm, B, Pmax, P_d, nm);
    if (c->front_stream && c->stream != c->front_stream) {
        HIPCHK(hipEventRecord(c->ev_mel_free, c->stream));
        c->mel_free_pending = true;
    }
    voc_conv_pre(c, v, vin, dom[0]);
    int Cin = c->voc_c0, rows = Pmax;
    for (int i = 0; i < ns; i++) {
        VocStage s;
        s.i = i; s.Cin = Cin; s.Cout = Cin / 2; s.rows_in = rows; s.rows = rows * c->voc_rates[i];
        s.len_in = v.lens_d + (size_t)(i + 1) * B; s.len = v.lens_d + (size_t)(i + 2) * B;
        s.dt_in = dom[i]; s.dt = dom[i + 1];
        s.next_slope = (i == ns - 1) ? 0.01f : 0.1f;
        c->tag = "voc.up" + std::to_string(i + 1);
        voc_upsample(c, v, s);
        c->tag = "voc.res" + std::to_string(i + 1);
        if (!voc_narrow_stage(c, v, s)) {
            if (v.side_ok) voc_side_begin(c);
            for (int j = 0; j < nk; j++) voc_resblock(c, v, s, j);
        }
        Cin = s.Cout; rows = s.rows;
    }
    c->tag = "voc.post";
    {
        double nout = 0; for (int b = 0; b < B; b++) nout += (double)mel_len_host[b] * c->hop;
        int nmax = 0; for (int b = 0; b < B; b++) nmax = std::max(nmax, mel_len_host[b] * c->hop);
        if ((long)nmax > wav_stride) nmax = (int)wav_stride;
        const int kp = c->t("voc.post_w").dim(0);
        c->timed(2.0 * nout * Cin * kp, nout * (Cin * es + (pcm16 ? 2.0 : 4.0)), [&] {
            launch_conv_post_tanh(v.A, dom[ns], Cin, (long)rows * Cin, c->pf("voc.post_w"), c->t("voc.post_b").host[0], kp,
                                  Cin, wav_dev, wav_stride, pcm16, B, nmax, P_d, c->hop, mel_len_d, c->hop, c->stream);
        });
    }
    c->tag = "other";
}

float* spkemb_from_mels(zvx_ctx* c, const float* mels_d, const int32_t* lens, int B, int Tmax) {
    const int dt = c->dt, F0 = c->n_mels, H = c->H;
    const size_t es = c->es();
    std::vector<int> W(4 * (size_t)B);
    int Wmax[4] = {Tmax, 0, 0, 0};
    for (int b = 0; b < B; b++) { int w = lens[b]; for (int l = 0; l < 4; l++) { W[(size_t)l * B + b] = w; w = (w - 1) / 2 + 1; } }
    for (int l = 1; l < 4; l++) Wmax[l] = (Wmax[l - 1] - 1) / 2 + 1;
    int WS[4]; for (int l = 0; l < 4; l++) WS[l] = Wmax[l] + 1;
    int Fh[4]; Fh[0] = F0; for (int l = 1; l < 4; l++) Fh[l] = (Fh[l - 1] - 1) / 2 + 1;
    int* W_d = c->upload_ints("spk.W", W.data(), W.size());

    const int C0 = c->rn_filters[0];
    size_t maxel = 0;
    for (int l = 0; l < 4; l++) maxel = std::max(maxel, (size_t)B * Fh[l] * WS[l] * c->rn_filters[l]);
    void* mA = c->buf("spk.mA", maxel * es); void* mB = c->buf("spk.mB", maxel * es);
    void* mC = c->buf("spk.mC", maxel * es); void* mD = c->buf("spk.mD", maxel * es);
    float* mean = c->fbuf("spk.mean", (size_t)B * 256 * 16); float* rstd = c->fbuf("spk.rstd", (size_t)B * 256 * 16);
    float* sescale = c->fbuf("spk.sescale", (size_t)B * 1024);

// ... 879 lines not shown
        wstride = (std::max(need, 1) + 7) & ~7;
        const size_t bytes = (size_t)B * wstride * ss;
        if (bytes > hs->cap) {
            if (hs->p) { HIPCHK(hipHostFree(hs->p)); hs->p = nullptr; hs->cap = 0; }
            const size_t cap = bytes + bytes / 8 + 256;
            HIPCHK(hipHostMalloc(&hs->p, cap, hipHostMallocDefault));
            hs->cap = cap;
        }
        wdev = c->buf(slot ? "wav.async1" : "wav.async0", bytes);
        hs->B = B; hs->pcm16 = pcm16; hs->stride = wstride; hs->need = need;
    } else if (dev_out) {
        wdev = wav; wstride = wav_stride;
        auto f = c->gather_fence.find(wav);
        if (f != c->gather_fence.end()) HIPCHK(hipStreamWaitEvent(c->stream, f->second, 0));
    }
    else { wstride = (std::max(need, 1) + 7) & ~7; wdev = c->buf("wav", (size_t)B * wstride * ss); }
    if (rs) {
        const long nstride = (std::max(need_native, 1) + 7) & ~7;
        float* native = c->fbuf("wav.native", (size_t)B * nstride);
        run_vocoder(c, c->fbuf("mel", 0), c->n_mels, c->Lmax, c->mel_len_host.data(), P.data(), B, native, nstride, 0);
        c->stage_end(ZVX_T_VOCODER);
        run_resample(c, *bank, native, nstride, c->ibuf("voc.lens", 0), c->hop, B, wdev, wstride, pcm16, plan);
    } else {
        run_vocoder(c, c->fbuf("mel", 0), c->n_mels, c->Lmax, c->mel_len_host.data(), P.data(), B, wdev, wstride, pcm16);
        c->stage_end(ZVX_T_VOCODER);
    }
    if (host_async) {
        HIPCHK(hipEventRecord(hs->ready, c->stream));
        HIPCHK(hipStreamWaitEvent(c->copy_stream, hs->ready, 0));
        if (need > 0) HIPCHK(hipMemcpyAsync(hs->p, wdev, (size_t)B * wstride * ss, hipMemcpyDeviceToHost, c->copy_stream));
        HIPCHK(hipEventRecord(hs->done, c->copy_stream));
        hs->pending = true;
        return;
    }
    if (!dev_out && need > 0)
        HIPCHK(hipMemcpy2DAsync(wav, (size_t)wav_stride * ss, wdev, (size_t)wstride * ss, (size_t)need * ss, B, hipMemcpyDeviceToHost, c->stream));
    if (!(dev_out && (flags & ZVX_NO_SYNC))) c->sync();
}

template <typename F>
zvx_status guarded(zvx_ctx* ctx, F&& f) {
    if (!ctx) return ZVX_E_INVALID;
    try {
        HIPCHK(hipSetDevice(ctx->device));
        const bool outer = ctx->api_depth++ == 0;
        struct End { zvx_ctx* c; ~End() { try { if (--c->api_depth == 0) c->arena_end(); } catch (...) {} } } end{ctx};
        if (outer) ctx->arena_begin();
        f();
        return ZVX_OK;
    } catch (const ZvxError& e) {
        ctx->err = e.what();
        ctx->quiesce_side_streams();
        return e.code;
    } catch (const std::exception& e) {
        ctx->err = e.what();
        ctx->quiesce_side_streams();
        return ZVX_E_INVALID;
    }
}

}

extern "C" {

zvx_status zvx_create(const char* manifest, const void* weights, size_t nbytes, int device, zvx_ctx** out) {
    if (!out) return ZVX_E_INVALID;
    *out = nullptr;
    zvx_ctx* c = new zvx_ctx();
    try {
        int ndev = 0;
        hipError_t e = hipGetDeviceCount(&ndev);
        if (e != hipSuccess || ndev <= 0) fail(ZVX_E_HIP, "no HIP device available (%s)", hipGetErrorString(e));
        if (device < 0 || device >= ndev) fail(ZVX_E_INVALID, "device %d out of range (%d visible)", device, ndev);
        c->device = device;
        HIPCHK(hipSetDevice(device));
        HIPCHK(hipStreamCreate(&c->stream));
        c->main0 = c->stream;
        for (int s = 0; s < ZVX_T_COUNT; s++) { HIPCHK(hipEventCreate(&c->stage_ev[s][0])); HIPCHK(hipEventCreate(&c->stage_ev[s][1])); c->stage_used[s] = false; c->stage_ms[s] = 0.f; }
        parse_manifest(c, manifest, weights, nbytes);
        read_config(c);
        upload_weights(c);
        *out = c;
        return ZVX_OK;
    } catch (const ZvxError& e) {
        g_create_error = e.what();
        delete c;
        return e.code;
    } catch (const std::exception& e) {
        g_create_error = e.what();
        delete c;
        return ZVX_E_INVALID;
    }
}

void zvx_destroy(zvx_ctx* c) {
    if (!c) return;
    (void)hipSetDevice(c->device);
    if (c->front_stream) (void)hipStreamSynchronize(c->front_stream);
    if (c->stream) (void)hipStreamSynchronize(c->stream);
    zvx_comm_destroy(c);
    for (int i = 0; i < 2; i++) { if (c->arena[i].p) (void)hipHostFree(c->arena[i].p); if (c->arena[i].ev) (void)hipEventDestroy(c->arena[i].ev); }
    if (c->copy_stream && !c->copy_is_comm) { (void)hipStreamSynchronize(c->copy_stream); (void)hipStreamDestroy(c->copy_stream); }
    for (auto& hs : c->host_slot) { if (hs.p) (void)hipHostFree(hs.p); if (hs.ready) (void)hipEventDestroy(hs.ready); if (hs.done) (void)hipEventDestroy(hs.done); }
    if (c->join_host) (void)hipHostFree(c->join_host);
    for (int i = 0; i < 2; i++) if (c->voc_aux[i]) { (void)hipStreamSynchronize(c->voc_aux[i]); (void)hipStreamDestroy(c->voc_aux[i]); }
    for (int i = 0; i < 3; i++) if (c->voc_ev[i]) (void)hipEventDestroy(c->voc_ev[i]);
    if (c->aux_stream) { (void)hipStreamSynchronize(c->aux_stream); (void)hipStreamDestroy(c->aux_stream); (void)hipEventDestroy(c->ev_aux[0]); (void)hipEventDestroy(c->ev_aux[1]); }
    if (c->front_stream) {
        (void)hipStreamSynchronize(c->front_stream); (void)hipStreamDestroy(c->front_stream);
        (void)hipEventDestroy(c->ev_front_done); (void)hipEventDestroy(c->ev_mel_free); (void)hipEventDestroy(c->ev_main_join);
    }
    for (auto& kv : c->bufs) if (kv.second.base) (void)hipFree(kv.second.base);
    for (auto e : c->event_pool) (void)hipEventDestroy(e);
    if (c->stream) {
        for (int s = 0; s < ZVX_T_COUNT; s++) { (void)hipEventDestroy(c->stage_ev[s][0]); (void)hipEventDestroy(c->stage_ev[s][1]); }
        (void)hipStreamDestroy(c->stream);
    }
    delete c;
}

const char* zvx_last_error(const zvx_ctx* c) { return c ? c->err.c_str() : g_create_error.c_str(); }

namespace {

struct Switch { const char* key; int zvx_ctx::*v; bool (*ok)(int64_t); };
bool flag(int64_t v) { return v == 0 || v == 1; }
bool count(int64_t v) { return v >= 0 && v <= INT32_MAX; }
const Switch kSwitches[] = {
    {"profile", &zvx_ctx::profile, [](int64_t v) { return v >= 0 && v <= 2; }},
    {"profile_only", &zvx_ctx::profile_only, [](int64_t v) { return v >= -1 && v < gemm_num_variants(); }},
    {"shape_log", &zvx_ctx::shape_log, flag},
    {"rs_prof", &zvx_ctx::rs_prof, flag},
    {"f16_sat_check", &zvx_ctx::sat_check, flag},
    {"poison_pads", &zvx_ctx::poison_pads, flag},
    {"max_frames", &zvx_ctx::max_frames, [](int64_t v) { return v >= 1 && v <= (1 << 24); }},
    {"enc_split", &zvx_ctx::enc_split, [](int64_t v) { return v >= 0 && v <= 2; }},
    {"attn_f32", &zvx_ctx::use_attn_f32, flag},
    {"flash", &zvx_ctx::use_flash, flag},
    {"front_overlap", &zvx_ctx::front_overlap, [](int64_t v) { return v >= 0 && v <= 2; }},
    {"va_overlap_maxb", &zvx_ctx::va_overlap_maxb, count},
    {"dec_f16", &zvx_ctx::dec_f16, flag},
    {"dec_flat", &zvx_ctx::dec_flat, flag},
    {"dec_sc_fuse", &zvx_ctx::dec_sc_fuse, flag},
    {"norm_fuse_maxb", &zvx_ctx::norm_fuse_maxb, count},
    {"voc_f16", &zvx_ctx::voc_f16, flag},
    {"voc_f16_stages", &zvx_ctx::voc_f16_stages, [](int64_t v) { return v >= -1 && v <= INT32_MAX; }},
    {"voc_overlap_maxb", &zvx_ctx::voc_overlap_maxb, count},
    {"voc_overlap_frames", &zvx_ctx::voc_overlap_frames, count},
    {"stagefuse", &zvx_ctx::use_stagefuse, flag},
    {"rb2fuse", &zvx_ctx::use_rb2fuse, flag},
    {"resstream", &zvx_ctx::use_resstream, flag},
    {"rs_seg_min", &zvx_ctx::rs_seg_min, [](int64_t v) { return v >= -1 && v <= INT32_MAX; }},
    {"pairstream", &zvx_ctx::use_pairstream, [](int64_t v) { return v == -1 || v == 0 || v == 1 || v == 3; }},
    {"slab_small", &zvx_ctx::slab_small, [](int64_t v) { return (v & ~32) >= 0 && (v & ~32) <= 2; }},
    {"slab_flat", &zvx_ctx::slab_flat, flag},
    {"spk_pool_fuse", &zvx_ctx::spk_pool_fuse, flag},
    {"spk_s2_fuse", &zvx_ctx::spk_s2_fuse, flag},
    {"out_rate", &zvx_ctx::out_rate, count},
};
const Switch* find_switch(const char* key) {
    for (const Switch& s : kSwitches) if (!strcmp(s.key, key)) return &s;
    return nullptr;
}

}

int64_t zvx_get_int(const zvx_ctx* c, const char* key) {
    if (!c || !key) return -1;
    if (const Switch* s = find_switch(key)) return c->*s->v;
    const std::string k(key);
    if (k == "precision") return c->dt == DT_F32 ? 1 : 0;
    if (k == "hidden") return c->H;
    if (k == "n_mels") return c->n_mels;
    if (k == "hop") return c->hop;
    if (k == "device") return c->device;
    if (k == "dec_kind") return c->dec_kind;
    if (k == "Lmax") return c->Lmax;
    if (k == "f16_sat_events") {
        zvx_ctx* m = const_cast<zvx_ctx*>(c);
        unsigned long long n = 0;
        if (hipSetDevice(m->device) != hipSuccess) return -1;
        try { unsigned long long* d = m->sat_count_dev(); m->sync(); if (hipMemcpy(&n, d, sizeof n, hipMemcpyDeviceToHost) != hipSuccess) return -1; } catch (...) { return -1; }
        return (int64_t)n;
    }
    if (k == "host_slot") return c->host_last;
    if (k.rfind("variant_id:", 0) == 0) { for (int i = 0; i < gemm_num_variants(); i++) if (k.substr(11) == gemm_variant_name(i)) return i; return -1; }
    auto it = c->cfg.find(k);
    if (it != c->cfg.end()) return atoll(it->second.c_str());
    return -1;
}

zvx_status zvx_set_int(zvx_ctx* c, const char* key, int64_t value) {
    return guarded(c, [&] {
        if (!key) fail(ZVX_E_INVALID, "key is NULL");
        const Switch* s = find_switch(key);
        if (!s) fail(ZVX_E_INVALID, "unknown option '%s'", key);
        if (!s->ok(value)) fail(ZVX_E_INVALID, "option '%s' does not take the value %lld", key, (long long)value);
        const std::string k(key);
        if (k == "out_rate" && value) {
            int L = 1, M = 1;
            rs_pair(model_rate(c), (int)value, &L, &M);
            if ((int)value != model_rate(c)) rs_bank(c, L, M);
        }
        if (k == "profile" || k == "profile_only" || k == "f16_sat_check" || k == "front_overlap") c->sync();
        c->*s->v = (int)value;
        if (k == "f16_sat_check") HIPCHK(hipMemsetAsync(c->sat_count_dev(), 0, 64, c->stream));
        if (k == "front_overlap") c->front_dirty_main = true;
        if (k == "enc_split") {
            if (c->dt != DT_BF16) c->enc_split = 0;
            if (c->enc_split) { c->sync(); build_split_weights(c, c->enc_split == 2); }
        }
    });
}

zvx_status zvx_spkemb(zvx_ctx* c, const float* ref_mels, const int32_t* lens, int B, int Tmax, float* out) {
    return guarded(c, [&] {
        if (!ref_mels || !lens || !out || B <= 0 || Tmax <= 0) fail(ZVX_E_INVALID, "zvx_spkemb: bad arguments");
        run_spkemb(c, ref_mels, lens, B, Tmax, out, 0);
    });
}

zvx_status zvx_spkemb_ex(zvx_ctx* c, const float* ref_mels, const int32_t* lens, int B, int Tmax, float* out, int flags) {
    return guarded(c, [&] {
        if (!ref_mels || !lens || !out || B <= 0 || Tmax <= 0) fail(ZVX_E_INVALID, "zvx_spkemb_ex: bad arguments");
        run_spkemb(c, ref_mels, lens, B, Tmax, out, flags);
    });
}

zvx_status zvx_melspec(zvx_ctx* c, const float* wav, const int32_t* nsamples, int B, int Nmax, float* mel, int Tmax, int32_t* frames) {
    return guarded(c, [&] {
        if (!wav || !nsamples || B <= 0 || Nmax <= 0 || Tmax <= 0) fail(ZVX_E_INVALID, "zvx_melspec: bad arguments");
        run_melspec(c, wav, nsamples, B, Nmax, mel, Tmax, frames);
    });
}

zvx_status zvx_spkemb_wav(zvx_ctx* c, const float* wav, const int32_t* nsamples, int B, int Nmax, int rate, const zvx_ref_params* params, float* out,
                          int32_t* begin, int32_t* end, int32_t* frames, int flags) {
    return guarded(c, [&] { do_spkemb_wav(c, wav, nsamples, B, Nmax, rate, params, out, begin, end, frames, flags); });
}

zvx_status zvx_encode(zvx_ctx* c, const int32_t* phoneme, const int32_t* puncts, const int32_t* duration, const int32_t* T,
                      int B, int Tmax, const float* spk, int32_t* mel_len, float* log_duration, float* pitch, float* energy) {
    return zvx_encode_ex(c, phoneme, puncts, duration, T, B, Tmax, spk, mel_len, log_duration, pitch, energy, nullptr);
}

zvx_status zvx_encode_ex(zvx_ctx* c, const int32_t* phoneme, const int32_t* puncts, const int32_t* duration, const int32_t* T,
                         int B, int Tmax, const float* spk, int32_t* mel_len, float* log_duration, float* pitch, float* energy,
                         const zvx_prosody* prosody) {
    return guarded(c, [&] {
        if (!phoneme || !puncts || !T || !spk) fail(ZVX_E_INVALID, "zvx_encode: NULL input");
        run_encode(c, phoneme, puncts, duration, T, B, Tmax, spk, mel_len, 0, prosody);
        const size_t nid = (size_t)B * Tmax;
        if (log_duration) HIPCHK(hipMemcpyAsync(log_duration, c->fbuf("va.logd", nid), nid * 4, hipMemcpyDeviceToHost, c->stream));
        if (pitch) HIPCHK(hipMemcpyAsync(pitch, c->fbuf("va.pitch", nid), nid * 4, hipMemcpyDeviceToHost, c->stream));
        if (energy) HIPCHK(hipMemcpyAsync(energy, c->fbuf("va.energy", nid), nid * 4, hipMemcpyDeviceToHost, c->stream));
        c->sync();
    });
}

zvx_status zvx_decode(zvx_ctx* c, float* mel_out, int Lstride, int flags) {
    return guarded(c, [&] {
        if (!c->have_features) fail(ZVX_E_STATE, "zvx_decode: no features in the context (call zvx_encode first)");
        const int B = c->B;
        int* L_d = c->upload_ints("dec.L", c->mel_len_host.data(), B);
        run_decode(c, c->fbuf("features", 0), c->fbuf("in.spk", 0), L_d, B, c->Lmax);
        if (mel_out && c->Lmax > 0) copy_out_rows(c, c->fbuf("mel", 0), c->Lmax, c->n_mels, mel_out, Lstride, B, flags & ZVX_DEVICE_OUT);
        c->sync();
    });
}

zvx_status zvx_decode_features(zvx_ctx* c, const float* features, const int32_t* L, int B, int Lmax, const float* spk,
                               float* mel_out, int Lstride) {
    return guarded(c, [&] {
        if (!features || !L || !spk || B <= 0 || Lmax <= 0) fail(ZVX_E_INVALID, "zvx_decode_features: bad arguments");
        for (int b = 0; b < B; b++) if (L[b] < 2 || L[b] > Lmax) fail(ZVX_E_INVALID, "L[%d]=%d out of range (2..%d)", b, L[b], Lmax);
        c->B = B; c->Lmax = Lmax; c->mel_len_host.assign(L, L + B); c->Tmax = 0;
        c->have_features = false; c->have_mel = false;
        float* f = c->fbuf("features", (size_t)B * Lmax * c->H);
        HIPCHK(hipMemcpyAsync(f, features, (size_t)B * Lmax * c->H * 4, hipMemcpyHostToDevice, c->stream));
        float* spk_d = c->fbuf("in.spk", (size_t)B * c->H);
        HIPCHK(hipMemcpyAsync(spk_d, spk, (size_t)B * c->H * 4, hipMemcpyHostToDevice, c->stream));
        int* L_d = c->upload_ints("dec.L", L, B);
        c->have_features = true;
        run_decode(c, f, spk_d, L_d, B, Lmax);
        if (mel_out) copy_out_rows(c, c->fbuf("mel", 0), Lmax, c->n_mels, mel_out, Lstride, B, false);
        c->sync();
    });
}

zvx_status zvx_vocode(zvx_ctx* c, const int32_t* pad_to, void* wav, int64_t wav_stride, int flags) {
    return guarded(c, [&] {
        if (!wav && !(flags & ZVX_HOST_ASYNC)) fail(ZVX_E_INVALID, "zvx_vocode: wav is NULL");
        do_vocode(c, pad_to, wav, wav_stride, flags);
    });
}

zvx_status zvx_vocode_mel(zvx_ctx* c, const float* mel, const int32_t* P, int B, int Pmax, void* wav, int64_t wav_stride, int flags) {
    return guarded(c, [&] {
        if (!mel || !P || (!wav && !(flags & ZVX_HOST_ASYNC)) || B <= 0 || Pmax <= 0) fail(ZVX_E_INVALID, "zvx_vocode_mel: bad arguments");
        for (int b = 0; b < B; b++) if (P[b] < 1 || P[b] > Pmax) fail(ZVX_E_INVALID, "P[%d]=%d out of range (1..%d)", b, P[b], Pmax);
        c->B = B; c->Lmax = Pmax; c->Tmax = 0; c->mel_len_host.assign(P, P + B);
        c->have_features = false; c->have_mel = false;
        float* m = c->fbuf("mel", (size_t)B * Pmax * c->n_mels);
        HIPCHK(hipMemcpyAsync(m, mel, (size_t)B * Pmax * c->n_mels * 4, (flags & ZVX_DEVICE_IN) ? hipMemcpyDeviceToDevice : hipMemcpyHostToDevice, c->stream));
        c->have_mel = true;
        do_vocode(c, nullptr, wav, wav_stride, flags);
// ... 385 lines not shown
```

### zerovox_amd/csrc/zvx_kernels.h

```cpp
#pragma once
#include <hip/hip_runtime.h>
#include <hip/hip_ext.h>
#include <stdint.h>
#include <atomic>
#include <mutex>
#include <set>
#include <utility>

extern thread_local hipEvent_t zvx_gemm_ev_start, zvx_gemm_ev_stop;
#define ZVX_DISPATCH(kernel, grid, block, lds, stream, ...) \
    do { if (zvx_gemm_ev_start) hipExtLaunchKernelGGL(kernel, grid, block, lds, stream, zvx_gemm_ev_start, zvx_gemm_ev_stop, 0, __VA_ARGS__); \
         else hipLaunchKernelGGL(kernel, grid, block, lds, stream, __VA_ARGS__); } while (0)

namespace zvx {

inline void profile_events(hipEvent_t start, hipEvent_t stop) { zvx_gemm_ev_start = start; zvx_gemm_ev_stop = stop; }

typedef unsigned short bf16_t;

enum DType { DT_F32 = 0, DT_BF16 = 1, DT_F16 = 2 };
static inline size_t dtype_size(int dt) { return dt == DT_F32 ? 4 : 2; }
inline int num_cus() {
    static const int n = [] { int dev = 0, v = 0; if (hipGetDevice(&dev) != hipSuccess || hipDeviceGetAttribute(&v, hipDeviceAttributeMultiprocessorCount, dev) != hipSuccess || v <= 0) v = 256; return v; }();
    return n;
}
inline int persistent_cus() { return num_cus(); }

inline bool lds_opt_in(const void* kfn) {
    static std::mutex mu;
    static std::set<std::pair<const void*, int>> done;
    int dev = 0;
    if (hipGetDevice(&dev) != hipSuccess) return false;
    std::lock_guard<std::mutex> lk(mu);
    if (done.count({kfn, dev})) return true;
    if (hipFuncSetAttribute(kfn, hipFuncAttributeMaxDynamicSharedMemorySize, 160 * 1024) != hipSuccess) return false;
    done.insert({kfn, dev});
    return true;
}

enum Act { ACT_NONE = 0, ACT_RELU = 1, ACT_LRELU = 2, ACT_TANH = 3 };

#define ZVX_MAX_TAPS 16

struct GemmArgs {
    const void* X; long x_bs, x_hs; int ldx;
    const void* W; long w_bs, w_hs, w_ts; int ldw;
    const void* Wp;
    int halo_l, halo_r;
    const void* Wp2; const float* bias1; int dv1[ZVX_MAX_TAPS]; int fused; float slope1;
    int no_pairstream;
    int dtype;
    int M, N, K;
    int nbatch, nheads;
    const int* in_len;
    const int* out_len;
    const int* k_len;
    int in_len_static;
    int ntaps; int du[ZVX_MAX_TAPS], dv[ZVX_MAX_TAPS];
    int stride, wout, hin, win;
    int flat_win, flat_rows;
    int bflat;
    const void* X2; long x2_bs; int ldx2, K2;
    int xcd_flat;
    int slab_small;
    int out_split3;
    float alpha;
    const float* bias; int bias_mode;
    const void* res; long r_bs, r_hs; int ldr; int res_dtype; int res_mode;
    float res_inv_slope;
    void* accum; long a_bs; int lda; int accum_mode;
    int accum_dtype;
    float out_scale;
    int act; float slope;
    const float* post_scale; const float* post_shift;
    void* out; long o_bs, o_hs; int ldo; int out_dtype;
    float* se_part; int* se_part_S;
    void* ds_out; const void* ds_Wp; const float* ds_bias;
    double flops;
};

int launch_gemm(const GemmArgs& a, hipStream_t stream);
int gemm_variant_of(const GemmArgs& a);
int gemm_epi_mode_of(const GemmArgs& a);
int launch_resfuse(GemmArgs a, hipStream_t stream);
int launch_rb2fuse(GemmArgs a, hipStream_t stream);
size_t packed_weight_elems(int ntaps, int N, int K);
void launch_pack_pair(const void* packedA, int ntapsA, int KA, const void* packedB, int ntapsB, int KB, int N, void* out, hipStream_t s);
void launch_pack_weights(const void* w_bf16, int ntaps, int N, int K, void* out, hipStream_t s);
const char* gemm_variant_name(int id);
int gemm_num_variants();

struct StreamArgs {
    const void* X; long x_bs; int ldx;
    const void* W1[3]; const void* W2[3];
    const float* b1[3]; const float* b2[3];
    int dil[3];
    int C, ntaps, npair;
    void* out; long o_bs; int ldo;
    void* accum; long a_bs; int lda; int accum_mode;
    float slope1, res_inv_slope, out_scale, slope;
    const int* len; int M, nbatch;
    int S, nseg;
    int dX0, dT, dX[3];
    double flops;
    long long* prof;
    int seg_min;
    int f16;
};
int launch_resstream(StreamArgs a, hipStream_t stream, bool dry_run);

struct PairArgs {
    const void* X; long x_bs; int ldx;
    const void* W1; const void* W2;
    const float* b1; const float* b2;
    int C, ntaps, dil;
    void* out; long o_bs; int ldo;
    void* accum; long a_bs; int lda; int accum_mode;
    float slope1, res_inv_slope, out_scale, slope;
    const int* len; int M, nbatch;
    int force;
    int f16;
    int S, nseg, DX, DT, G0;
    long long* prof;
};
bool launch_pairstream(PairArgs a, hipStream_t stream, bool dry_run);

struct StageArgs {
    const void* X; long x_bs; int ldx;
    const void* W;
    int woff[18];
    const float* bias;
    int C, nk, ks[3], dil[3][3];
    void* out; long o_bs; int ldo;
    float slope1, res_inv_slope, slope;
    const int* len; int M, nbatch;
    int f16;
};
bool launch_narrowstage(const StageArgs& a, hipStream_t stream, bool dry_run);
int narrowstage_steps(int C, int k);
void launch_pack_narrow(const void* w16 , int k, int C, void* out, hipStream_t s);

struct FlashArgs {
    const void* qk; long qk_bs; int ldq; int k_off;
    const void* vt; long vt_bs; int ldv;
    void* out; long o_bs; int ldo;
    const int* len; int L, D, nheads, nbatch;
    float scale;
    int f16;
    long long* prof;
};
bool launch_flash_attention(const FlashArgs& a, hipStream_t stream, bool dry_run);
struct AttnF32Args {
    const float* qkv; long bs; int ld; int q_off, k_off, v_off;
    float* out; long o_bs; int ldo;
    unsigned short* planes; int planes_C;
    int planes_f16;
    const int* len; int L, D, nheads, nbatch;
    float scale;
};
bool launch_attention_f32(const AttnF32Args& a, hipStream_t stream, bool dry_run);

void launch_instnorm_fused(const void* x, int x_dt, int ldx, void* y, int y_dt, int ldy, int B, int Lmax, const int* L, int C, float eps,
                           float* mean, float* rstd, const float* gamma, const float* beta, long g_bs, int one_plus, int act, float slope, hipStream_t s);
void launch_transpose16(const void* in, int ld_in, void* out, int ld_out, int B, int rows, int C, hipStream_t s, const int* len = nullptr);
void launch_f32_to_bf16(const float* in, bf16_t* out, size_t n, hipStream_t s);
void launch_zero_tail_cols(void* x, int es, long ld, long bs, int B, int rows, int cols, const int* len, hipStream_t s);
void launch_cast(const void* in, int in_dt, void* out, int out_dt, size_t n, hipStream_t s);

void launch_split3(const float* x, int ldx, void* out, int B, int rows_max, const int* rows, int C, hipStream_t s, int f16 = 0);
void launch_split3_weights(const float* w, void* out, long nrows, int K, hipStream_t s, int f16 = 0, float scale = 1.f);
void launch_absmax(const float* x, size_t n, float* out , hipStream_t s);

void launch_embed(const int* phoneme, const int* puncts, const float* emb, int emb_dim, const float* pemb,
                  int pemb_dim, const float* pe, float* out, int B, int Tmax, const int* T, hipStream_t s);

void launch_layernorm(const void* x, int x_dt, int ldx, void* y, int y_dt, int ldy, int B, int rows_max,
                      const int* rows, int C, int mode, float eps, const float* gamma, const float* beta,
                      const float* bg, long bg_bs, const float* post_add, hipStream_t s, void* split_planes = nullptr, int planes_f16 = 0);

void launch_softmax_rows(const float* scores, int lds, void* P, int p_dt, int ldp, int nbatch, int nheads,
                         int Lmax, const int* len, hipStream_t s);

void launch_rowdot(const float* x, int ldx, const float* w, float bias, float* out, int B, int Tmax,
                   const int* T, int C, hipStream_t s);

void launch_bucket_embed_add(const float* pred, const float* table, int nbins, float* x, int ldx, int C,
                             int* idx_out, int B, int Tmax, const int* T, hipStream_t s);

void launch_durations(const int* forced, const float* logd, int* dur, int* cum, int* mel_len, int B, int Tmax,
                      const int* T, hipStream_t s);

void launch_bucket_embed_add_ctl(const float* pred, const float* shift, const float* range, const float* target, const float* table,
                                 int nbins, float* x, int ldx, int C, int* idx_out, int B, int Tmax, const int* T, hipStream_t s);
void launch_durations_q16(const int* forced, const float* logd, const int* q, int* dur, int* cum, int* mel_len, int B, int Tmax,
                          const int* T, hipStream_t s);

void launch_length_regulate(const float* x, int ldx, const int* cum, const int* T, const int* mel_len,
                            float* feats, int B, int Tmax, int Lmax, int C, hipStream_t s);
void launch_add_pe_cast(const float* x, const float* pe, void* y, int y_dt, int ldy, int B, int Lmax,
                        const int* L, int C, hipStream_t s, int out_rows_max = 0);

void launch_instnorm_stats(const void* x, int x_dt, int ldx, int B, int Lmax, const int* L, int C, float eps,
                           float* mean, float* rstd, hipStream_t s);
void launch_norm_affine_act(const void* x, int x_dt, int ldx, void* y, int y_dt, int ldy, int B, int Lmax,
                            const int* L, int C, const float* mean, const float* rstd, const float* gamma,
                            const float* beta, long g_bs, int one_plus, int act, float slope, hipStream_t s);

void launch_mel_pad(const void* mel, int m_dt, int ldm, int Lmax, const int* mel_len, void* v, int v_dt,
                    int ldv, int Pmax, const int* P, int B, int nm, hipStream_t s);
void launch_copy_rows_f32(const void* src, int s_dt, int lds, long s_bs, float* dst, long ldd, long d_bs,
                          int B, int rows_max, const int* rows, int C, hipStream_t s);

void launch_conv_post_tanh(const void* x, int x_dt, int ldx, long x_bs, const float* w , float bias,
                           int ktaps, int C, void* wav, long wav_bs, int pcm16, int B, int Nmax, const int* in_len,
                           int len_mul, const int* out_len, int out_mul, hipStream_t s);
struct ResampleArgs {
    const float* x; long x_bs; const int* in_len; int in_mul;
// ... 102 lines not shown
```

Baseline: 353.3 million.

## Add 16x16x32 MFMA path to conv slab kernel for vocoder resblock GEMMs

Adds an S16 variant of the conv slab kernel that uses 16x16x32 f16/bf16 MFMA instructions with f32x4 accumulators instead of the 32x32 tiles. This needs a new LDS pitch, different lane-to-row/K mapping, paired weight loads and an epilogue adapter for the new accumulator layout. The path is enabled through a flag bit for vocoder resblock 1x1 GEMMs with at least 256 channels, and a wide_mfma switch controls it. The aim is higher MFMA throughput and better pipelining on MI355X, at the cost of more instructions per tile, larger LDS pitch and a risky new data mapping.

```diff
diff --git a/zerovox_amd/csrc/gemm.hip b/zerovox_amd/csrc/gemm.hip
--- a/zerovox_amd/csrc/gemm.hip
+++ b/zerovox_amd/csrc/gemm.hip
@@ -278,12 +278,27 @@
 #define ZVX_EPI_DEC(res) (16 | 8 | (res))
 #define ZVX_EPI_FLIP (ZVX_EPI(0, 0, 1) | 32)
 
-template <int TM, int TN, int RES_LDS = 0, int EPI = -1, bool H16 = false>
-__device__ __forceinline__ void epilogue_rows(const GemmArgs& a, f32x16 (&acc)[TN][TM], int b, int row_base, int col_base,
+template <class T> struct acc_is16 { static constexpr bool value = false; };
+template <int A, int B> struct acc_is16<f32x4[A][B]> { static constexpr bool value = true; };
+template <int TN, int TM>
+__device__ __forceinline__ float4 acc_quad(const f32x16 (&acc)[TN][TM], int i, int j, int g) {
+    return make_float4(acc[i][j][4 * g], acc[i][j][4 * g + 1], acc[i][j][4 * g + 2], acc[i][j][4 * g + 3]);
+}
+template <int TN2, int TM2>
+__device__ __forceinline__ float4 acc_quad(const f32x4 (&acc)[TN2][TM2], int i, int j, int g) {
+    const f32x4 v = acc[2 * i + (g >> 1)][2 * j + (g & 1)];
+    return make_float4(v[0], v[1], v[2], v[3]);
+}
+template <bool S16> __device__ __forceinline__ int acc_row(int lane, int g) { return S16 ? 16 * (g & 1) + (lane & 15) : (lane & 31); }
+template <bool S16> __device__ __forceinline__ int acc_chan(int lane, int g) { return S16 ? 16 * (g >> 1) + 4 * (lane >> 4) : 8 * g + 4 * (lane >> 5); }
+
+template <int TM, int TN, int RES_LDS = 0, int EPI = -1, bool H16 = false, class ACC>
+__device__ __forceinline__ void epilogue_rows(const GemmArgs& a, ACC& acc, int b, int row_base, int col_base,
                                               int out_len, int lane, unsigned char* stage ,
                                               const unsigned char* res_lds = nullptr ,
                                               int res_pitch = 0) {
     constexpr int NW = TN * 32;
+    constexpr bool S16 = acc_is16<ACC>::value;
     constexpr int EP = NW * 4 + 16;
     constexpr int LPR = NW / 8;
     constexpr int RPP = 64 / LPR;
@@ -329,8 +344,7 @@
         for (int i = 0; i < TN; i++)
 #pragma unroll
             for (int g = 0; g < 4; g++)
-                *(float4*)(stage + (lane & 31) * EP + (i * 32 + 8 * g + 4 * (lane >> 5)) * 4) =
-                    make_float4(acc[i][j][4 * g], acc[i][j][4 * g + 1], acc[i][j][4 * g + 2], acc[i][j][4 * g + 3]);
+                *(float4*)(stage + acc_row<S16>(lane, g) * EP + (i * 32 + acc_chan<S16>(lane, g)) * 4) = acc_quad(acc, i, j, g);
         f32x2 v[NP][4];
         uint4 rraw[NP];
         float4 aa0[NP], aa1[NP];
@@ -469,19 +483,20 @@
 #undef pk2
 }
 
-template <int TM, int TN, bool F16 = false>
-__device__ __forceinline__ void epilogue_direct(const GemmArgs& a, f32x16 (&acc)[TN][TM], int b, int row_base, int col_base,
+template <int TM, int TN, bool F16 = false, class ACC>
+__device__ __forceinline__ void epilogue_direct(const GemmArgs& a, ACC& acc, int b, int row_base, int col_base,
                                                 int out_len, int lane, unsigned char* stage ) {
     constexpr int NW = TN * 32, EP = NW * 2 + 16, LPR = NW / 8, RPP = 64 / LPR, NP = 32 / RPP;
+    constexpr bool S16 = acc_is16<ACC>::value;
     const float slope = a.act == ACT_LRELU ? a.slope : 1.f;
-    const int h4 = 4 * (lane >> 5), c8 = lane % LPR, n = col_base + c8 * 8;
+    const int c8 = lane % LPR, n = col_base + c8 * 8;
     const bool nok = n < a.N;
     float4 bb[TN][4];
 #pragma unroll
     for (int i = 0; i < TN; i++)
 #pragma unroll
         for (int g = 0; g < 4; g++) {
-            const int co = col_base + i * 32 + 8 * g + h4;
+            const int co = col_base + i * 32 + acc_chan<S16>(lane, g);
             bb[i][g] = co < a.N ? *(const float4*)(a.bias + co) : make_float4(0.f, 0.f, 0.f, 0.f);
         }
     unsigned short* obase = (unsigned short*)a.out + (long)b * a.o_bs + n;
@@ -492,12 +507,13 @@
         for (int i = 0; i < TN; i++)
 #pragma unroll
             for (int g = 0; g < 4; g++) {
-                const f32x2 v01 = lrelu2((f32x2){acc[i][j][4 * g], acc[i][j][4 * g + 1]} + (f32x2){bb[i][g].x, bb[i][g].y}, slope);
-                const f32x2 v23 = lrelu2((f32x2){acc[i][j][4 * g + 2], acc[i][j][4 * g + 3]} + (f32x2){bb[i][g].z, bb[i][g].w}, slope);
+                const float4 q = acc_quad(acc, i, j, g);
+                const f32x2 v01 = lrelu2((f32x2){q.x, q.y} + (f32x2){bb[i][g].x, bb[i][g].y}, slope);
+                const f32x2 v23 = lrelu2((f32x2){q.z, q.w} + (f32x2){bb[i][g].z, bb[i][g].w}, slope);
                 uint2 pk;
                 pk.x = pack16x2(v01.x, v01.y, F16);
                 pk.y = pack16x2(v23.x, v23.y, F16);
-                *(uint2*)(stage + (lane & 31) * EP + (i * 32 + 8 * g + h4) * 2) = pk;
+                *(uint2*)(stage + acc_row<S16>(lane, g) * EP + (i * 32 + acc_chan<S16>(lane, g)) * 2) = pk;
             }
 #pragma unroll
         for (int p = 0; p < NP; p++) o[j][p] = *(const u32x4*)(stage + (p * RPP + lane / LPR) * EP + c8 * 16);
@@ -514,6 +530,7 @@
 #if ZVX_PART_MAIN
 #define SLAB_KC 64
 #define SLAB_PITCH 144
+#define SLAB_PITCH16 160
 
 __global__ void k_pack_w(const unsigned short* w, int ntaps, int N, int K, unsigned short* out, int nkc, long total_frag_lanes) {
     long idx = (long)blockIdx.x * blockDim.x + threadIdx.x;
@@ -554,9 +571,11 @@
     (void)hipMemcpy2DAsync((char*)out + szA, szA + szB, packedB, szB, szB, nt, hipMemcpyDeviceToDevice, s);
 }
 
-template <int BM, int BN, int WM, int WN, bool FULLK, int MINW, int R, int EPI = -1, int MAXH = 64, bool F16 = false>
+template <int BM, int BN, int WM, int WN, bool FULLK, int MINW, int R, int EPI = -1, int MAXH = 64, bool F16 = false, bool S16 = false>
 __global__ __launch_bounds__(256, MINW) void convslab_kernel(const GemmArgs a) {
     constexpr int TM = BM / WM / 32, TN = BN / WN / 32;
+    constexpr int SPITCH = S16 ? SLAB_PITCH16 : SLAB_PITCH;
+    static_assert(!S16 || FULLK, "16x16x32 steps: whole K chunks");
     constexpr int NIT = ((BM + MAXH) * 8 + 255) / 256;
     static_assert(WM * WN == 4, "4 waves");
     extern __shared__ __attribute__((aligned(16))) unsigned char slab[];
@@ -609,13 +628,21 @@
         }
     }
 
-    f32x16 acc[TN][TM];
-#pragma unroll
-    for (int i = 0; i < TN; i++)
-#pragma unroll
-        for (int j = 0; j < TM; j++)
-#pragma unroll
-            for (int e = 0; e < 16; e++) acc[i][j][e] = 0.f;
+    f32x16 acc[S16 ? 1 : TN][S16 ? 1 : TM];
+    f32x4 acc4[S16 ? 2 * TN : 1][S16 ? 2 * TM : 1];
+    if (S16) {
+#pragma unroll
+        for (int i = 0; i < 2 * TN; i++)
+#pragma unroll
+            for (int j = 0; j < 2 * TM; j++) acc4[S16 ? i : 0][S16 ? j : 0] = (f32x4){0.f, 0.f, 0.f, 0.f};
+    } else {
+#pragma unroll
+        for (int i = 0; i < TN; i++)
+#pragma unroll
+            for (int j = 0; j < TM; j++)
+#pragma unroll
+                for (int e = 0; e < 16; e++) acc[S16 ? 0 : i][S16 ? 0 : j][e] = 0.f;
+    }
 
     constexpr bool WREG = R == 0;
     constexpr int F = BN / 32, CNT = F >= 4 ? F / 4 : 1, WD = 4, D = WREG ? WD : R - 1, WAITN = WREG ? (WD - 1) * TN : (D - 2) * CNT;
@@ -627,9 +654,9 @@
         const int f = wave * CNT + j, t32 = (n0 >> 5) + f;
         wsrc[j] = (const uint4*)a.Wp + (long)(t32 < nt32_total ? t32 : 0) * gtotal * 64 + lane;
     }
-    const int xrow0 = HL + wr * (BM / WM) + (lane & 31);
-    const int koff = (lane >> 5) * 16;
-    unsigned char* ring = slab + ((SR * SLAB_PITCH + 1023) & ~1023);
+    const int xrow0 = HL + wr * (BM / WM) + (S16 ? (lane & 15) : (lane & 31));
+    const int koff = S16 ? (lane >> 4) * 16 : (lane >> 5) * 16;
+    unsigned char* ring = slab + ((SR * SPITCH + 1023) & ~1023);
     const unsigned lds_base = (unsigned)(size_t)(__attribute__((address_space(3))) unsigned char*)slab;
     const int dvreg = a.dv[lane & (ZVX_MAX_TAPS - 1)];
     const bool loader = wave * CNT < F;
@@ -640,13 +667,22 @@
         wq[i] = (const unsigned char*)a.Wp + (long)(t32 < nt32_total ? t32 : 0) * gtotal * 1024;
     }
     const bool wave_dead = __builtin_amdgcn_readfirstlane((int)(n0 + wc * TN * 32 >= a.N)) != 0;
-    const unsigned lane16 = lane * 16;
+    const unsigned lane16 = S16 ? (lane >> 5) * 1024 + ((lane & 15) + 32 * ((lane >> 4) & 1)) * 16 : lane * 16;
     u32x4 wreg[WREG ? WD : 1][TN] = {};
     auto wload = [&](int gs, int slot) {
         const long off = (long)(gs < gtotal ? gs : gtotal - 1) * 1024;
 #pragma unroll
         for (int i = 0; i < TN; i++)
             asm volatile("global_load_dwordx4 %0, %1, %2" : "+v"(wreg[WREG ? slot : 0][i]) : "v"(lane16), "s"(wq[i] + off) : "memory");
+    };
+    auto wload16 = [&](int grp, int par) {
+        if (!(S16 && WREG)) return;
+        const long off = (long)(grp < (gtotal >> 1) ? grp : (gtotal >> 1) - 1) * 2048;
+#pragma unroll
+        for (int i = 0; i < TN; i++) {
+            asm volatile("global_load_dwordx4 %0, %1, %2" : "+v"(wreg[(S16 && WREG) ? 2 * par : 0][i]) : "v"(lane16), "s"(wq[i] + off) : "memory");
+            asm volatile("global_load_dwordx4 %0, %1, %2 offset:256" : "+v"(wreg[(S16 && WREG) ? 2 * par + 1 : 0][i]) : "v"(lane16), "s"(wq[i] + off) : "memory");
+        }
     };
     auto dma = [&](int gs) {
         if (WREG || !loader) return;
@@ -657,7 +693,8 @@
             __builtin_amdgcn_global_load_lds((const __attribute__((address_space(1))) void*)(wsrc[j] + off),
                                              (__attribute__((address_space(3))) void*)(ring + (slot * F + wave * CNT + j) * 1024), 16, 0, 0);
     };
-    if (WREG) { wload(0, 0); wload(1, 1); wload(2, 2); wload(3, 3); }
+    if (S16 && WREG) { wload16(0, 0); wload16(1, 1); }
+    else if (WREG) { wload(0, 0); wload(1, 1); wload(2, 2); wload(3, 3); }
     else {
 #pragma unroll
         for (int s0 = 0; s0 < D; s0++) dma(s0);
@@ -685,7 +722,7 @@
 #pragma unroll
                 for (int i = 0; i < FCH; i++) {
                     const int c = tid + (h0 + i) * 256;
-                    if (h0 + i < NIT && c < SR * 8) *(uint4*)(slab + (c >> 3) * SLAB_PITCH + (c & 7) * 16) = sv[i];
+                    if (h0 + i < NIT && c < SR * 8) *(uint4*)(slab + (c >> 3) * SPITCH + (c & 7) * 16) = sv[i];
                 }
             }
         }
@@ -706,7 +743,7 @@
             }
 #pragma unroll
             for (int j = 0; j < TM; j++)
-                asm volatile("ds_read_b128 %0, %1" : "=v"(xf[j]) : "v"(lds_base + rowoff + j * 32 * SLAB_PITCH + kk * 32));
+                asm volatile("ds_read_b128 %0, %1" : "=v"(xf[j]) : "v"(lds_base + rowoff + j * 32 * SPITCH + kk * 32));
         };
         auto mma = [&](uint4 (&xf)[TM], uint4 (&wf)[TN]) {
 #pragma unroll
@@ -728,9 +765,64 @@
         };
         auto rowoff_of = [&](int tap) {
             const int d = src2 ? 0 : __builtin_amdgcn_readlane(dvreg, tap < ntaps ? tap : ntaps - 1);
-            return (unsigned)((xrow0 + d) * SLAB_PITCH + koff);
+            return (unsigned)((xrow0 + d) * SPITCH + koff);
         };
         unsigned rowoff = rowoff_of(0);
+        auto rd16 = [&](uint4 (&xf)[TM], unsigned ro, int st) {
+#pragma unroll
+            for (int j = 0; j < TM; j++)
+                asm volatile("ds_read_b128 %0, %1" : "=v"(xf[j]) : "v"(lds_base + ro + ((st & 1) * TM + j) * 16 * SPITCH + (st >> 1) * 64));
+        };
+        uint4 w16A[2 * TN], w16B[2 * TN];
+        const unsigned ring_rd16 = lds_base + (unsigned)(size_t)(ring - slab) + wc * TN * 1024 + (lane >> 5) * (F * 1024) + ((lane & 15) + 32 * ((lane >> 4) & 1)) * 16;
+        auto rdw16 = [&](uint4 (&wf)[2 * TN], int gs_even) {
+            const unsigned wa = ring_rd16 + (gs_even & ((WREG ? 1 : R) - 1)) * (F * 1024);
+#pragma unroll
+            for (int i = 0; i < TN; i++) {
+                asm volatile("ds_read_b128 %0, %1 offset:%2" : "=v"(wf[2 * i]) : "v"(wa), "n"(i * 1024));
+                asm volatile("ds_read_b128 %0, %1 offset:%2" : "=v"(wf[2 * i + 1]) : "v"(wa), "n"(i * 1024 + 256));
+            }
+        };
+        auto mma16 = [&](uint4 (&xf)[TM], int st) {
+#pragma unroll
+            for (int i = 0; i < TN; i++)
+#pragma unroll
+                for (int h = 0; h < 2; h++)
+#pragma unroll
+                    for (int j = 0; j < TM; j++) {
+                        f32x4& c4 = acc4[S16 ? 2 * i + h : 0][S16 ? (st & 1) * TM + j : 0];
+                        const u32x4 wv = WREG ? wreg[(S16 && WREG) ? 2 * (st >> 1) + h : 0][i] : __builtin_bit_cast(u32x4, (st >> 1) ? w16B[2 * i + h] : w16A[2 * i + h]);
+                        c4 = F16 ? __builtin_amdgcn_mfma_f32_16x16x32_f16(__builtin_bit_cast(f16x8, wv), __builtin_bit_cast(f16x8, xf[j]), c4, 0, 0, 0)
+                                 : __builtin_amdgcn_mfma_f32_16x16x32_bf16(__builtin_bit_cast(bf16x8, wv), __builtin_bit_cast(bf16x8, xf[j]), c4, 0, 0, 0);
+                    }
+        };
+        if (S16) {
+            if (!WREG) rdw16(w16A, gs0);
+            rd16(xA, rowoff, 0);
+            for (int tap = 0; tap < ntaps_kc; tap++) {
+                const unsigned rowoff_next = rowoff_of(tap + 1);
+                const int grp = (gs0 >> 1) + tap * 2;
+#pragma unroll
+                for (int st = 0; st < 4; st++) {
+                    const int gs = gs0 + tap * 4 + st;
+                    if (WREG) asm volatile("s_waitcnt vmcnt(%0)" :: "n"(2 * TN) : "memory");
+                    else if (st & 1) asm volatile("s_waitcnt vmcnt(%0)\n\ts_barrier" :: "n"(WAITN - CNT) : "memory");
+                    else asm volatile("s_waitcnt vmcnt(%0)\n\ts_barrier" :: "n"(WAITN) : "memory");
+                    dma(gs + D);
+                    if (!WREG && st == 1) rdw16(w16B, gs + 1);
+                    if (!WREG && st == 3) rdw16(w16A, gs + 1);
+                    if (st & 1) rd16(xA, st == 3 ? rowoff_next : rowoff, (st + 1) & 3);
+                    else        rd16(xB, rowoff, st + 1);
+                    if (!WREG && (st & 1)) asm volatile("s_waitcnt lgkmcnt(%0)" :: "n"(TM + 2 * TN) : "memory");
+                    else asm volatile("s_waitcnt lgkmcnt(%0)" :: "n"(TM) : "memory");
+                    __builtin_amdgcn_sched_barrier(0);
+                    if (st & 1) mma16(xB, st); else mma16(xA, st);
+                    __builtin_amdgcn_sched_barrier(0);
+                    if (WREG && (st & 1)) wload16(grp + (st >> 1) + 2, st >> 1);
+                }
+                rowoff = rowoff_next;
+            }
+        } else {
         rd(xA, wA, gs0, rowoff, 0);
         for (int tap = 0; tap < ntaps_kc; tap++) {
             const unsigned rowoff_next = rowoff_of(tap + 1);
@@ -753,6 +845,7 @@
             }
             rowoff = rowoff_next;
         }
+        }
         asm volatile("s_waitcnt lgkmcnt(0)" ::: "memory");
     }
     if (WREG) {
@@ -764,12 +857,15 @@
         asm volatile("s_waitcnt vmcnt(0)" ::: "memory");
     }
     __syncthreads();
-    if (EPI == ZVX_EPI_FLIP)
-        epilogue_direct<TM, TN, !F16>(a, acc, b, m0 + wr * (BM / WM), n0 + wc * (BN / WN), out_len, lane, slab + wave * (32 * (TN * 64 + 16)));
-    else if (EPI == ZVX_EPI(0, 0, 1))
-        epilogue_direct<TM, TN, F16>(a, acc, b, m0 + wr * (BM / WM), n0 + wc * (BN / WN), out_len, lane, slab + wave * (32 * (TN * 64 + 16)));
-    else
-        epilogue_rows<TM, TN, 0, EPI, (F16 && EPI >= 0)>(a, acc, b, m0 + wr * (BM / WM), n0 + wc * (BN / WN), out_len, lane, slab + wave * (32 * (TN * 32 * 4 + 16)));
+    auto finish = [&](auto& tile) {
+        if (EPI == ZVX_EPI_FLIP)
+            epilogue_direct<TM, TN, !F16>(a, tile, b, m0 + wr * (BM / WM), n0 + wc * (BN / WN), out_len, lane, slab + wave * (32 * (TN * 64 + 16)));
+        else if (EPI == ZVX_EPI(0, 0, 1))
+            epilogue_direct<TM, TN, F16>(a, tile, b, m0 + wr * (BM / WM), n0 + wc * (BN / WN), out_len, lane, slab + wave * (32 * (TN * 64 + 16)));
+        else
+            epilogue_rows<TM, TN, 0, EPI, (F16 && EPI >= 0)>(a, tile, b, m0 + wr * (BM / WM), n0 + wc * (BN / WN), out_len, lane, slab + wave * (32 * (TN * 32 * 4 + 16)));
+    };
+    if constexpr (S16) finish(acc4); else finish(acc);
 }
 
 template <int C, int NT, int BM, int WM, int WN, int MINW, int MAXH = 64, bool F16 = false>
@@ -1742,9 +1838,14 @@
 int gemm_num_variants() { return (int)(sizeof(kVariants) / sizeof(kVariants[0])); }
 
 
-template <int BM, int BN, int WM, int WN, int MINW, int R, int EPI = -1>
+template <int BM, int BN, int WM, int WN, int MINW, int R, int EPI = -1, bool S16 = false>
 static void launch_slab_variant(const GemmArgs& a, dim3 grid, size_t lds, hipStream_t stream) {
     const bool fullk = a.K % SLAB_KC == 0 && a.K2 == 0;
+    if constexpr (S16) {
+        if (a.dtype == DT_F16) ZVX_LAUNCH((convslab_kernel<BM, BN, WM, WN, true, MINW, R, EPI, 64, true, true>), grid, dim3(256), lds, stream, a);
+        else ZVX_LAUNCH((convslab_kernel<BM, BN, WM, WN, true, MINW, R, EPI, 64, false, true>), grid, dim3(256), lds, stream, a);
+        return;
+    }
     if constexpr (R == 0 || EPI == -1 || EPI == ZVX_EPI(0, 0, 1) || EPI == ZVX_EPI_FLIP) {
         if (a.dtype == DT_F16) {
             if (fullk) ZVX_LAUNCH((convslab_kernel<BM, BN, WM, WN, true, MINW, R, EPI, 64, true>), grid, dim3(256), lds, stream, a);
@@ -1778,6 +1879,12 @@
     return -1;
 }
 
+static bool slab_s16_of(const GemmArgs& a) {
+    if (!(a.slab_small & ZVX_SLAB_S16) || a.dtype == DT_F32 || a.K % SLAB_KC || a.K2 || a.flat_win || a.bflat) return false;
+    const int e = gemm_epi_mode_of(a);
+    return e < 0 || !(e & (16 | 32));
+}
+
 static int launch_convslab(GemmArgs a, hipStream_t stream) {
     const bool bflat_hint = a.bflat != 0;
     if (a.K2) {
@@ -1834,6 +1941,8 @@
         }
         return -4;
     }
+    const bool s16 = slab_s16_of(a);
+    const size_t pitch = s16 ? SLAB_PITCH16 : SLAB_PITCH;
     static const int bns[4] = {256, 128, 64, 32};
     static const double eff[4] = {0.95, 1.0, 0.7, 0.4};
     int best = 0; double best_cost = -1;
@@ -1846,8 +1955,9 @@
     if (g_slab_small >= 2 && a.M <= 64 && a.nbatch * ((a.N + 127) / 128) * 4 <= ncu && a.N >= 64 && hl + hr <= 64) {
         a.bflat = 0;
         dim3 g32((a.N + 31) / 32, a.nbatch);
-        const size_t lds32 = (((size_t)(256 + hl + hr) * SLAB_PITCH + 1023) & ~(size_t)1023) + (size_t)8 * 1024;
-        launch_slab_variant<256, 32, 4, 1, 2, 8>(a, g32, lds32, stream);
+        const size_t lds32 = (((size_t)(256 + hl + hr) * pitch + 1023) & ~(size_t)1023) + (size_t)8 * 1024;
+        if (s16) launch_slab_variant<256, 32, 4, 1, 2, 8, -1, true>(a, g32, lds32, stream);
+        else launch_slab_variant<256, 32, 4, 1, 2, 8>(a, g32, lds32, stream);
         return 9;
     }
     if (g_slab_small && a.M > 128 && a.N >= 128 && hl + hr <= 64) {
@@ -1857,10 +1967,13 @@
             const bool r64 = wg256 * 4 <= ncu;
             const int bm = r64 ? 64 : 128;
             dim3 gs(((a.N + 127) / 128) * ((a.M + bm - 1) / bm), a.nbatch);
-            size_t lds = ((size_t)(bm + hl + hr) * SLAB_PITCH + 1023) & ~(size_t)1023;
+            size_t lds = ((size_t)(bm + hl + hr) * pitch + 1023) & ~(size_t)1023;
             const size_t stage = (size_t)4 * 32 * (2 * 128 + 16);
             if (lds < stage) lds = stage;
-            if (r64) launch_slab_variant<64, 128, 2, 2, 2, 0>(a, gs, lds, stream);
+            if (s16) {
+                if (r64) launch_slab_variant<64, 128, 2, 2, 2, 0, -1, true>(a, gs, lds, stream);
+                else launch_slab_variant<128, 128, 2, 2, 2, 0, -1, true>(a, gs, lds, stream);
+            } else if (r64) launch_slab_variant<64, 128, 2, 2, 2, 0>(a, gs, lds, stream);
             else launch_slab_variant<128, 128, 2, 2, 2, 0>(a, gs, lds, stream);
             return 22;
         }
@@ -1871,16 +1984,22 @@
         const bool narrow = wide < 2 * ncu;
         const int bn = narrow ? 128 : 256;
         dim3 grid((a.N + bn - 1) / bn, a.nbatch);
-        size_t lds = ((size_t)(128 + hl + hr) * SLAB_PITCH + 1023) & ~(size_t)1023;
+        size_t lds = ((size_t)(128 + hl + hr) * pitch + 1023) & ~(size_t)1023;
         const size_t stage = (size_t)4 * 32 * (2 * 128 + 16);
         if (lds < stage) lds = stage;
         if (narrow && a.M > (g_slab_small ? 32 : 64) && ((a.N + 127) / 128) * a.nbatch < 2 * ncu) {
             dim3 g64(((a.N + 127) / 128) * ((a.M + 63) / 64), a.nbatch);
-            launch_slab_variant<64, 128, 2, 2, 2, 0>(a, g64, lds, stream);
+            if (s16) launch_slab_variant<64, 128, 2, 2, 2, 0, -1, true>(a, g64, lds, stream);
+            else launch_slab_variant<64, 128, 2, 2, 2, 0>(a, g64, lds, stream);
             return 22;
         }
-        if (narrow) { launch_slab_variant<128, 128, 2, 2, 2, 0>(a, grid, lds, stream); return 22; }
-        launch_slab_variant<128, 256, 1, 4, 2, 0>(a, grid, lds, stream);
+        if (narrow) {
+            if (s16) launch_slab_variant<128, 128, 2, 2, 2, 0, -1, true>(a, grid, lds, stream);
+            else launch_slab_variant<128, 128, 2, 2, 2, 0>(a, grid, lds, stream);
+            return 22;
+        }
+        if (s16) launch_slab_variant<128, 256, 1, 4, 2, 0, -1, true>(a, grid, lds, stream);
+        else launch_slab_variant<128, 256, 1, 4, 2, 0>(a, grid, lds, stream);
         return 6;
     }
     if (a.ntaps == 1 && a.N >= 512) {
@@ -1924,9 +2043,22 @@
     dim3 grid(ntn * ntm, a.nbatch);
     const int tn = (bn >= 128) ? 2 : 1;
     if (a.accum_mode && a.accum && a.accum_dtype == DT_F16 && tn == 2 && !(best == 1 && gemm_epi_mode_of(a) >= 0)) return -6;
-    size_t lds = (((size_t)(bm + hl + hr) * SLAB_PITCH + 1023) & ~(size_t)1023) + (size_t)ring_slots * (bn / 32) * 1024;
+    size_t lds = (((size_t)(bm + hl + hr) * pitch + 1023) & ~(size_t)1023) + (size_t)ring_slots * (bn / 32) * 1024;
     const size_t stage = (size_t)4 * 32 * (tn * 128 + 16);
     if (lds < stage) lds = stage;
+    if (s16 && best == 0) { launch_slab_variant<128, 256, 1, 4, 2, 0, -1, true>(a, grid, lds, stream); return 6; }
+    if (s16 && best == 3) { launch_slab_variant<256, 32, 4, 1, 2, 8, -1, true>(a, grid, lds, stream); return 9; }
+    if (s16 && best == 1) {
+        switch (gemm_epi_mode_of(a)) {
+            case ZVX_EPI(0, 0, 1): launch_slab_variant<256, 128, 2, 2, 2, 0, ZVX_EPI(0, 0, 1), true>(a, grid, lds, stream); break;
+            case ZVX_EPI(1, 0, 1): launch_slab_variant<256, 128, 2, 2, 2, 0, ZVX_EPI(1, 0, 1), true>(a, grid, lds, stream); break;
+            case ZVX_EPI(1, 2, 0): launch_slab_variant<256, 128, 2, 2, 2, 0, ZVX_EPI(1, 2, 0), true>(a, grid, lds, stream); break;
+            case ZVX_EPI(1, 3, 0): launch_slab_variant<256, 128, 2, 2, 2, 0, ZVX_EPI(1, 3, 0), true>(a, grid, lds, stream); break;
+            case ZVX_EPI(1, 1, 1): launch_slab_variant<256, 128, 2, 2, 2, 0, ZVX_EPI(1, 1, 1), true>(a, grid, lds, stream); break;
+            default: launch_slab_variant<256, 128, 2, 2, 2, 0, -1, true>(a, grid, lds, stream);
+        }
+        return 7;
+    }
     switch (best) {
         case 0: launch_slab_variant<128, 256, 1, 4, 2, 0>(a, grid, lds, stream); break;
         case 1: switch (gemm_epi_mode_of(a)) {
diff --git a/zerovox_amd/csrc/zvx.hip b/zerovox_amd/csrc/zvx.hip
--- a/zerovox_amd/csrc/zvx.hip
+++ b/zerovox_amd/csrc/zvx.hip
@@ -112,6 +112,7 @@
     int rs_seg_min = 0;
     int spk_s2_fuse = 1;
     int spk_pool_fuse = 1;
+    int wide_mfma = 1;
     int slab_small = 2, slab_flat = 1;
     int poison_pads = 0;
     int sat_check = 0;
@@ -266,7 +267,7 @@
     void gemm(GemmArgs& a) {
         if (a.flops <= 0) a.flops = 2.0 * (double)a.M * a.nbatch * a.nheads * (double)a.N * ((double)a.K * a.ntaps + (double)a.K2);
         if (!a.Wp && a.dtype != DT_F32) { auto it = packed.find(a.W); if (it != packed.end()) a.Wp = it->second; }
-        a.slab_small = slab_small | (spk_s2_fuse ? 0 : 32); a.xcd_flat = slab_flat;
+        a.slab_small = slab_small | (spk_s2_fuse ? 0 : 32) | (wide_mfma ? a.slab_small & ZVX_SLAB_S16 : 0); a.xcd_flat = slab_flat;
         profiled([&] { return gemm_variant_of(a); }, [&] {
             const int id = a.fused == 2 ? launch_rb2fuse(a, stream) : (a.fused ? launch_resfuse(a, stream) : launch_gemm(a, stream));
             if (id < 0) fail(ZVX_E_INVALID, "launch_gemm rejected shape M=%d N=%d K=%d taps=%d", a.M, a.N, a.K, a.ntaps);
@@ -1397,6 +1398,7 @@
         GemmArgs a = gemm_base(dt);
         a.M = rows; a.N = Cout; a.K = Cout; a.nbatch = B; a.in_len = s.len; a.out_len = s.len; a.ldw = Cout; a.w_ts = (long)Cout * Cout;
         a.x_bs = (long)rows * Cout; a.ldx = Cout; a.o_bs = (long)rows * Cout; a.ldo = Cout;
+        if (c->voc_resblock == 1 && dt != DT_F32 && Cout >= 256) a.slab_small = ZVX_SLAB_S16;
         return a;
     };
     if (c->voc_resblock == 2 && nd == 2 && dt != DT_F32 && c->use_rb2fuse && !c->sat_check && (Cout == 32 || Cout == 64) && w.c1[0].packed && w.c1[1].packed) {
@@ -2582,6 +2584,7 @@
     {"resstream", &zvx_ctx::use_resstream, flag},
     {"rs_seg_min", &zvx_ctx::rs_seg_min, [](int64_t v) { return v >= -1 && v <= INT32_MAX; }},
     {"pairstream", &zvx_ctx::use_pairstream, [](int64_t v) { return v == -1 || v == 0 || v == 1 || v == 3; }},
+    {"wide_mfma", &zvx_ctx::wide_mfma, flag},
     {"slab_small", &zvx_ctx::slab_small, [](int64_t v) { return (v & ~32) >= 0 && (v & ~32) <= 2; }},
     {"slab_flat", &zvx_ctx::slab_flat, flag},
     {"spk_pool_fuse", &zvx_ctx::spk_pool_fuse, flag},
diff --git a/zerovox_amd/csrc/zvx_kernels.h b/zerovox_amd/csrc/zvx_kernels.h
--- a/zerovox_amd/csrc/zvx_kernels.h
+++ b/zerovox_amd/csrc/zvx_kernels.h
@@ -63,6 +63,7 @@
     const void* X2; long x2_bs; int ldx2, K2;
     int xcd_flat;
     int slab_small;
+#define ZVX_SLAB_S16 64
     int out_split3;
     float alpha;
     const float* bias; int bias_mode;
```

Result: no change. 356.5 million (median of 6 runs) (+0.9%).
